# dojo-sim/ContactImplicitMPC.jl

Measured on AMD Instinct MI355X. Metric: MPC steps/s (quadruped, H=40, fp64), higher is better.
Workload: dtype f64

## Files before the change

### contactimplicitmpc/jl_amd/csrc/cimpc_host.cpp

```cpp
#include <hip/hip_runtime.h>

#include <algorithm>
#include <chrono>
#include <cmath>
#include <cstdio>
#include <cstdlib>
#include <cstring>
#include <string>
#include <vector>

#include "cimpc_internal.h"
#include "lin_table.h"
#include "lin_table_build.h"
#include "model_table.h"
#include "newton_state.h"
#include "gains.h"
#include "handle_state.h"
#include "plant_linearize.h"
#include "schedule_plan.h"

using namespace cimpc;

namespace {

thread_local std::string g_create_error;

enum ProfClass { PC_IP = 0, PC_KKT = 1, PC_RESID = 2, PC_OTHER = 3, PC_ASYNC = 4, PC_COUNT = 5 };

struct ProfRec {
    hipEvent_t a, b;
    int cls;
};

}

struct RoundStreams {
    hipStream_t st = nullptr;
    hipStream_t st_kkt = nullptr;
    hipEvent_t ev_join = nullptr;
    hipEvent_t ev_start = nullptr;
};

struct Knobs {
    SchedulePolicy sched{};
    bool async_debug = false;
    double watchdog_s = 30.0;
    bool debug_rounds = false;
    bool generic_static = false;
    KktPolicy kkt{};
    int kkt_tw_nb = 0;
    int kkt_tw_spins = 0;
    int banded_form = 0;

    static int env_int(const char* name, int dflt) { const char* v = getenv(name); return v ? atoi(v) : dflt; }
    void read_environment() {
        sched.async_mode = env_int("CIMPC_ASYNC", sched.async_mode);
        sched.async_tail = env_int("CIMPC_ASYNC_TAIL", sched.async_tail);
        sched.spec_first = env_int("CIMPC_SPEC_FIRST", sched.spec_first);
        sched.iter_cap = std::max(1, env_int("CIMPC_ITER_CAP", sched.iter_cap));
        async_debug = getenv("CIMPC_ASYNC_DEBUG") != nullptr;
        if (const char* v = getenv("CIMPC_ASYNC_WATCHDOG_S")) watchdog_s = atof(v);
        debug_rounds = getenv("CIMPC_DEBUG_ROUNDS") != nullptr;
        sched.tail_div = env_int("CIMPC_TAIL_DIV", sched.tail_div);
        sched.async_full_max = env_int("CIMPC_ASYNC_FULL_MAX", sched.async_full_max);
        sched.drain_pct = env_int("CIMPC_DRAIN_PCT", sched.drain_pct);
        sched.drain_min = std::max(1, env_int("CIMPC_DRAIN_MIN", sched.drain_min));
        kkt.kkt_pipe = env_int("CIMPC_KKT_PIPE", kkt.kkt_pipe);
        kkt.kkt_twisted = env_int("CIMPC_KKT_TWISTED", kkt.kkt_twisted);
        kkt_tw_nb = env_int("CIMPC_KKT_TW_NB", kkt_tw_nb);
        kkt.lazy_dz = env_int("CIMPC_LAZY_DZ", 1) != 0;
        kkt.kkt_duo = env_int("CIMPC_KKT_DUO", kkt.kkt_duo);
        kkt.kkt_duo_hint = env_int("CIMPC_KKT_DUO_HINT", kkt.kkt_duo_hint);
        kkt.async_kkt_tw = env_int("CIMPC_ASYNC_KKT_TW", kkt.async_kkt_tw);
        generic_static = env_int("CIMPC_GENERIC_STATIC", generic_static ? 1 : 0) != 0;
        sched.sweep_wgs = env_int("CIMPC_SWEEP_WGS", sched.sweep_wgs);
        sched.waves32 = env_int("CIMPC_WAVES32", sched.waves32);
        banded_form = env_int("CIMPC_BANDED_FORM", banded_form);
    }
};

struct cimpc_ctx {
    cimpc_dims dm{};
    Knobs kn{};
    cimpc_ip_opts ip{};
    cimpc_newton_opts nt{};
    int device = 0;
    hipStream_t stream = nullptr;
    bool own_stream = false;
    std::string err;
    KernelInfo ki{};
    int nz = 0, nth = 0, nths = 0, nd = 0, nr = 0, nx = 0, ny = 0, N = 0;
    std::vector<void*> allocs;
    double* d_tab = nullptr;
    IpQueues Q{};
    int* d_window = nullptr;
    double *g_q = nullptr, *g_u = nullptr, *g_w = nullptr, *g_g = nullptr, *g_b = nullptr, *g_th = nullptr, *g_stride = nullptr;
    int* g_phase = nullptr;
    int* d_good_src = nullptr;
    double* d_dz_knot = nullptr;
    double* d_alt = nullptr;
    double* d_zout = nullptr;
    double *d_Q = nullptr, *d_R = nullptr, *d_Qinv = nullptr, *d_Rinv = nullptr, *d_Cg = nullptr,
           *d_Cb = nullptr;
    double *d_q0 = nullptr, *d_q1 = nullptr;
    double* h_qin = nullptr;
    double* h_stage = nullptr;
    size_t h_stage_doubles = 0;
    double* d_result = nullptr;
    double* h_result = nullptr;
    double* d_rhs = nullptr;
    double* d_pstate = nullptr;
    long long ip_budget_ticks = 0;
    NewtonDev S{};
    int* h_counters = nullptr;
    std::vector<char> knot_set;
    int n_knots_set = 0;
    HandleState st;
    KktPolicy kp{};
    KktCaps kc{};
    KktBackend kb = KktBackend::Condensed;
    long long n_kkt_twisted = 0;
    int* h_twfail = nullptr;
    int twfail_seen = 0;
    long long n_kkt_tw_fallbacks = 0;
    bool band_reduce_ok = false;
    double* d_mix_ws = nullptr;
    int* d_mix_nfb = nullptr;
    size_t dense_ws_doubles = 0;
    bool cf_tiny = true;
    double* d_cf_ws = nullptr;
    double* d_dense_ws = nullptr;
    double *d_V = nullptr, *d_qt = nullptr, *d_vt = nullptr;
    int* d_ring = nullptr;
    size_t ctl_ints = 0;
    int* h_ring = nullptr;
    int* h_ring_dev = nullptr;
    SchedulePlan sched{};
    bool async_dirty = true;
    int* a_items = nullptr;
    int* a_jobs = nullptr;
    int* a_ctrl = nullptr;
    int* a_evals = nullptr;
    long long* a_dbg = nullptr;
    size_t a_cap = 0, a_rq_cap = 0, a_kq_cap = 0;
    RoundStreams rs;
    bool external_stream = false;
    std::vector<double> h_tab;
    std::vector<double> h_tab_work;
    double* d_tb = nullptr;
    size_t tb_cap = 0;
    double *d_gK = nullptr, *d_glatch = nullptr, *d_gio = nullptr;
    cimpc_stats last_stats{};
    int prof_on = 0;
    bool prof_open = false;
    std::vector<ProfRec> prof_recs;
    std::vector<hipEvent_t> ev_pool;
    double prof_ms[PC_COUNT] = {0, 0, 0, 0, 0};
    long long prof_n[PC_COUNT] = {0, 0, 0, 0, 0};
    long long prof_async_problems = 0;
    long long prof_ip_problems = 0, prof_kkt_systems = 0;
};

namespace {

int fail(cimpc_ctx* h, int code, const std::string& msg) {
    if (h) h->err = msg;
    else g_create_error = msg;
    return code;
}
int refuse(cimpc_ctx* h, const Refusal& r) { return r.code == CIMPC_OK ? CIMPC_OK : fail(h, r.code, r.msg); }

}

void cimpc::set_global_error(const std::string& msg) { g_create_error = msg; }

namespace {

#define HIP_TRY(h, call)                                                                     \
    do {                                                                                     \
        hipError_t e__ = (call);                                                             \
        if (e__ != hipSuccess)                                                               \
            return fail(h, CIMPC_ERR_HIP, std::string(#call) + ": " + hipGetErrorString(e__)); \
    } while (0)

template <class T>
int dev_alloc(cimpc_ctx* h, T** p, size_t count) {
    void* v = nullptr;
    if (count == 0) count = 1;
    hipError_t e = hipMalloc(&v, count * sizeof(T));
    if (e != hipSuccess) return fail(h, CIMPC_ERR_HIP, std::string("hipMalloc: ") + hipGetErrorString(e));
    e = hipMemset(v, 0, count * sizeof(T));
    if (e == hipSuccess) e = hipStreamSynchronize(nullptr);
    if (e != hipSuccess) return fail(h, CIMPC_ERR_HIP, std::string("hipMemset: ") + hipGetErrorString(e));
    h->allocs.push_back(v);
    *p = static_cast<T*>(v);
    return CIMPC_OK;
}

int table_layout(cimpc_ctx* h, LinLayout* L) {
    *L = LinLayout(h->nx, h->ny, h->nth, h->ki.G, h->ki.generic ? 0 : h->nths, h->ki.generic ? 0 : h->ki.adj);
    if (L->size != h->ki.tab_size) return fail(h, CIMPC_ERR_STATE, "table layout of the library and of the kernel differ");
    return CIMPC_OK;
}

void prof_begin(cimpc_ctx* h, int cls, hipStream_t st = nullptr) {
    h->prof_open = false;
    if (!h->prof_on || (h->prof_on == 2 && cls != PC_IP)) return;
    h->prof_open = true;
    if (!st) st = h->stream;
    ProfRec r;
    auto get = [&]() {
        if (!h->ev_pool.empty()) {
            hipEvent_t e = h->ev_pool.back();
            h->ev_pool.pop_back();
            return e;
        }
        hipEvent_t e;
        (void)hipEventCreate(&e);
        return e;
    };
    r.a = get();
    r.b = get();
    r.cls = cls;
    (void)hipEventRecord(r.a, st);
    h->prof_recs.push_back(r);
}
void prof_end(cimpc_ctx* h, hipStream_t st = nullptr) {
    if (!h->prof_on || !h->prof_open) return;
    h->prof_open = false;
    (void)hipEventRecord(h->prof_recs.back().b, st ? st : h->stream);
}
void prof_collect(cimpc_ctx* h) {
    if (h->prof_recs.empty()) return;
    (void)hipStreamSynchronize(h->stream);
    if (h->rs.st) (void)hipStreamSynchronize(h->rs.st);
    if (h->rs.st_kkt) (void)hipStreamSynchronize(h->rs.st_kkt);
    for (auto& r : h->prof_recs) {
        float ms = 0.f;
        if (hipEventElapsedTime(&ms, r.a, r.b) == hipSuccess) {
            h->prof_ms[r.cls] += ms;
            h->prof_n[r.cls] += 1;
        }
        h->ev_pool.push_back(r.a);
        h->ev_pool.push_back(r.b);
    }
    h->prof_recs.clear();
}

IpParams make_ip_params(cimpc_ctx* h, const TrajDev& T, int par, int* pending_counter, double* zout) {
    IpParams p{};
    p.tab = h->d_tab;
    p.Q = h->Q;
    p.Q.par = par;
    p.wpk = h->sched.wpk;
    p.q = T.q;
    p.theta = T.th;
    p.gam = T.g;
    p.bfr = T.b;
    p.alt = h->st.has_altitude() ? h->d_alt : nullptr;
    p.d = h->S.d;
    p.dz = h->S.dz;
    p.nu = nullptr; p.dtn = nullptr; p.dtn_ld = h->S.dtn_ld;
    p.status = h->S.ip_status;
    p.iters = h->S.ip_iters;
    p.zout = zout;
    p.pflag = h->S.pflag;
    p.pstate = h->d_pstate;
    p.pending_count = pending_counter;
    p.iter_cap = h->kn.sched.iter_cap;
    p.slots = CS;
    p.H = h->dm.H;
    p.o = h->ip;
    p.kc_floor = h->ip.kappa_tol / h->ip.undercut;
    p.tau_floor = 1.0 - h->ip.eps_min;
    p.reg_floor = h->ip.kappa_tol * h->ip.gamma_reg;
    p.budget_ticks = h->ip_budget_ticks;
    p.generic_static = h->kn.generic_static ? 1 : 0;
    return p;
}

int run_sweep(cimpc_ctx* h, int par, int* pending_counter, double* zout, hipStream_t st, int iter_cap = 0, int* drain_counter = nullptr,
              bool with_products = false, long long hint = -1) {
    IpParams p = make_ip_params(h, h->S.cand, par, pending_counter, zout);
    if (with_products && h->S.dtn != nullptr) { p.nu = h->S.nu_cand; p.dtn = h->S.dtn; }
    if (iter_cap > 0) p.iter_cap = iter_cap;
    const SweepLaunch l = plan_sweep(h->kn.sched, h->sched, hint, p.iter_cap, h->ip.max_iter, drain_counter != nullptr);
    p.wpk = l.wpk; p.direct = l.direct;
    if (l.drain_thresh > 0) { p.drain_count = drain_counter; p.drain_thresh = l.drain_thresh; p.drain_min = h->kn.sched.drain_min; }
    prof_begin(h, PC_IP, st);
    int rc = launch_ip_sweep(&h->dm, p, l.waves, st);
    prof_end(h, st);
    if (rc != CIMPC_OK) return fail(h, rc, "ip sweep launch failed");
    return CIMPC_OK;
}

static void set_kkt_backend(cimpc_ctx* h) {
    NewtonDev& S = h->S;
    KktCaps& c = h->kc;
    c.cfg = h->dm.mode == CIMPC_MODE_CONFIGURATION;
    c.velocity = S.V != nullptr;
    c.cf_tiny = h->cf_tiny;
    c.wide_tiles = (h->dm.nq > 16 || h->dm.nu > 16) && h->dm.nq <= 24 && h->dm.nu <= 24;
    c.condensed = kkt_condensed_available(S);
    c.mfma = kkt_mfma_available(S);
    c.packed = kkt_packed_available(S);
    c.twisted = kkt_twisted_available(S);
    c.duo = kkt_duo_available(S);
    c.mixed = kkt_mixed_available(S);
    auto pick_band_form = [&](auto avail) {
        for (int r = h->band_reduce_ok ? 1 : 0; r >= 0; --r) { S.band_reduce = r; if (avail()) return true; }
        S.band_reduce = h->band_reduce_ok ? 1 : 0;
        return false;
    };
    S.band_reduce = h->band_reduce_ok ? 1 : 0;
    c.banded = c.cfg && pick_band_form([&] { return kkt_banded_available(S); });
    c.cf_reduce = !c.cfg && (c.velocity ? pick_band_form([&] { return kkt_cf_reduce_available(S); }) : kkt_cf_reduce_available(S));
    c.banded_twisted = kkt_banded_twisted_available(c.cfg ? S : cf_shadow(S));
    h->kb = select_kkt_backend(c, h->nt.kkt_backend);
    S.good_src = kkt_lazy_commit(h->kp, c, h->kb) ? h->d_good_src : nullptr;
}

int ensure_kkt_ws(cimpc_ctx* h) {
    if (h->kb == KktBackend::Condensed) return CIMPC_OK;
    if (h->kb == KktBackend::CondensedMixed) {
        if (h->d_mix_ws) return CIMPC_OK;
        if (dev_alloc(h, &h->d_mix_ws, kkt_mixed_workspace_doubles(h->S)) != CIMPC_OK) return CIMPC_ERR_HIP;
        return dev_alloc(h, &h->d_mix_nfb, 1);
    }
    const bool cf = h->kb == KktBackend::CfCondensed || h->kb == KktBackend::CfBanded;
    if (cf && !h->d_cf_ws && dev_alloc(h, &h->d_cf_ws, cf_reduce_doubles(h->S)) != CIMPC_OK) return CIMPC_ERR_HIP;
    if (h->kb == KktBackend::CfCondensed) return CIMPC_OK;
    const size_t need = cf ? kkt_dense_workspace_doubles(cf_shadow(h->S), true) : kkt_dense_workspace_doubles(h->S, h->kb == KktBackend::Banded);
    if (h->d_dense_ws && h->dense_ws_doubles >= need) return CIMPC_OK;
    h->d_dense_ws = nullptr;
    h->dense_ws_doubles = need;
    return dev_alloc(h, &h->d_dense_ws, need);
}

static KktForm plan_kkt_stage(cimpc_ctx* h, const KktSite& site) {
    const KktForm f = choose_kkt_form(h->kp, h->kc, h->kb, site);
    if (two_ended(f)) h->n_kkt_twisted++;
    return f;
}
static int run_kkt_stage(cimpc_ctx* h, const NewtonDev& Sk, const KktArgs& K, const KktSite& site, const int* list, int n, const int* n_dev, hipStream_t st) {
    return launch_kkt_stage(Sk, K, h->kb, plan_kkt_stage(h, site), list, n, n_dev, KktWorkspace{h->d_dense_ws, h->d_cf_ws, h->d_mix_ws, h->d_mix_nfb}, st);
}

int read_stats(cimpc_ctx* h, long long out[4]) {
    std::vector<long long> v((size_t)h->dm.B * 4);
    HIP_TRY(h, hipMemcpy(v.data(), h->S.stats, v.size() * sizeof(long long), hipMemcpyDeviceToHost));
    out[0] = out[1] = out[2] = out[3] = 0;
    for (size_t b = 0; b < (size_t)h->dm.B; ++b)
        for (int k = 0; k < 4; ++k) out[k] += v[b * 4 + k];
    return CIMPC_OK;
}

int drain_pending(cimpc_ctx* h) {
    if (!h->st.drain_needed()) return CIMPC_OK;
    HIP_TRY(h, hipStreamSynchronize(h->stream));
    h->st.advance_drained();
    return CIMPC_OK;
}

int check_ready(cimpc_ctx* h, bool need_newton) {
    if (!h) return CIMPC_ERR_INVALID;
    return refuse(h, h->st.solve_refusal(h->n_knots_set == h->dm.H_ref, need_newton));
}

}

extern "C" {

int cimpc_version(void) { return 108; }

void cimpc_default_ip_opts(cimpc_ip_opts* o) {
    if (!o) return;
    o->r_tol = 1.0e-8;
    o->kappa_tol = 2.0e-4;
    o->undercut = 5.0;
    o->gamma_reg = 0.1;
    o->kappa_reg = 1.0e-3;
    o->eps_min = 0.05;
    o->ls_scale = 0.5;
    o->max_iter = 100;
    o->max_ls = 3;
    o->stall_alpha = 1.0e-13;
    o->max_time = 0.0;
}

void cimpc_default_newton_opts(cimpc_newton_opts* o) {
    if (!o) return;
    o->r_tol = 3.0e-4;
    o->beta_init = 1.0e-5;
    o->max_time = 0.0;
    o->kappa = 2.0e-4;
    o->max_iter = 5;
    o->kkt_backend = CIMPC_KKT_CONDENSED;
}

const char* cimpc_last_error(cimpc_handle h) { return h ? h->err.c_str() : g_create_error.c_str(); }

int cimpc_create(const cimpc_dims* dims, const cimpc_ip_opts* ip, const cimpc_newton_opts* nt,
                 int device, cimpc_handle* out) {
    if (!dims || !out) return fail(nullptr, CIMPC_ERR_INVALID, "null argument");
    *out = nullptr;
    const cimpc_dims& d = *dims;
    if (d.nq <= 0 || d.nu < 0 || d.nw < 0 || d.nc <= 0 || d.nb < 0 || d.H <= 0 || d.H_ref <= 0 ||
        d.B <= 0 || (d.mode != 0 && d.mode != 1))
        return fail(nullptr, CIMPC_ERR_INVALID, "invalid dimensions");
    int ndev = 0;
    if (hipGetDeviceCount(&ndev) != hipSuccess || ndev <= 0)
        return fail(nullptr, CIMPC_ERR_NO_DEVICE,
                    "no HIP device visible: this library has no CPU fallback");
    if (device < 0 || device >= ndev) return fail(nullptr, CIMPC_ERR_NO_DEVICE, "device index out of range");
    hipDeviceProp_t prop;
    if (hipGetDeviceProperties(&prop, device) != hipSuccess)
        return fail(nullptr, CIMPC_ERR_NO_DEVICE, "hipGetDeviceProperties failed");
    if (std::strncmp(prop.gcnArchName, "gfx950", 6) != 0)
        return fail(nullptr, CIMPC_ERR_NO_DEVICE,
                    std::string("device is ") + prop.gcnArchName + ", kernels are built for gfx950 only");
    if (hipSetDevice(device) != hipSuccess) return fail(nullptr, CIMPC_ERR_NO_DEVICE, "hipSetDevice failed");

    cimpc_ctx* h = new cimpc_ctx();
    h->dm = d;
    if (ip) h->ip = *ip; else cimpc_default_ip_opts(&h->ip);
    if (nt) h->nt = *nt; else cimpc_default_newton_opts(&h->nt);
    h->device = device;
    if (h->ip.max_time > 0.0 && h->ip.max_time < 1000.0) {
        if (h->ip.max_iter >= 128) { delete h; return fail(nullptr, CIMPC_ERR_INVALID, "ip max_time needs max_iter < 128 (the parked state packs both into one word)"); }
        int khz = 0;
        if (hipDeviceGetAttribute(&khz, hipDeviceAttributeWallClockRate, device) != hipSuccess || khz <= 0) {
            delete h;
            return fail(nullptr, CIMPC_ERR_HIP, "ip max_time: the device does not report hipDeviceAttributeWallClockRate");
        }
        h->ip_budget_ticks = std::max<long long>(1, (long long)std::llround(h->ip.max_time * 1.0e3 * (double)khz));
    }
    h->kn.read_environment();
    if (ip_kernel_info(&h->dm, &h->ki) != CIMPC_OK) {
        delete h;
        std::string built;
        for (const ModelRow& r : MODEL_TABLE) (built += built.empty() ? "" : ", ") += r.name;
        return fail(nullptr, CIMPC_ERR_INVALID, "model dimensions outside the runtime-dimension kernel (nx, ny <= 64) and without a compiled set (built: " + built + ")");
    }
    h->nx = d.nq;
    h->ny = 2 * d.nc + d.nb;
    h->nz = d.nq + 4 * d.nc + 2 * d.nb;
    h->nth = 2 * d.nq + d.nu + d.nw + 2;
    h->nths = 2 * d.nq + d.nu;
    h->nd = d.mode ? d.nq + d.nc + d.nb : d.nq;
    h->nr = d.mode ? d.nq + d.nu + d.nc + d.nb : d.nq + d.nu;
    h->N = d.H * (h->nr + h->nd);
    if (hipStreamCreateWithFlags(&h->stream, hipStreamNonBlocking) != hipSuccess) {
        delete h;
        return fail(nullptr, CIMPC_ERR_HIP, "hipStreamCreate failed");
    }
    h->own_stream = true;
    h->knot_set.assign(d.H_ref, 0);
    h->h_tab.assign(h->ki.tab_size, 0.0);
    h->h_tab_work.assign(lin_table_work_doubles(h->nx, h->ny), 0.0);

    const size_t B = d.B, H = d.H;
    int rc = CIMPC_OK;
    {
        const size_t K = d.H_ref;
        const size_t evals = 1 + 7 * (size_t)std::max(1, h->nt.max_iter);
        h->a_cap = B * evals * ((H + K - 1) / K + 1);
        h->a_rq_cap = B * (2 + 3 * (size_t)std::max(1, h->nt.max_iter));
        h->a_kq_cap = B * (2 + 3 * (size_t)std::max(1, h->nt.max_iter));
        const size_t bytes = (K * h->a_cap + h->a_rq_cap + h->a_kq_cap) * sizeof(int);
        h->sched = plan_schedule(h->kn.sched, ScheduleFacts{d.B, d.H, d.H_ref, h->ki.G, newton_async_available(&d) && K <= 256 && bytes <= ((size_t)1 << 30)});
    }
    auto A = [&](auto** p, size_t n) { if (rc == CIMPC_OK) rc = dev_alloc(h, p, n); };
    A(&h->d_tab, (size_t)d.H_ref * h->ki.tab_size);
    {
        const size_t K = d.H_ref;
        const size_t cap = B * CS * ((H + K - 1) / K + 1);
        h->Q.K = (int)K; h->Q.cap = (int)cap; h->Q.par = 0;
        A(&h->Q.items, 2 * K * cap);
        const QueueCtl L = queue_ctl(K);
        h->ctl_ints = L.ints;
        A(&h->Q.count, h->ctl_ints);
        if (rc == CIMPC_OK) { h->Q.head = h->Q.count + L.head; h->d_ring = h->Q.count + L.counters; }
        A(&h->Q.done_count, B * CS);
        A(&h->d_window, B * (H + 2));
        h->Q.window = h->d_window;
    }
    A(&h->d_alt, B * d.nc);
    A(&h->d_zout, B * CS * H * h->nz);
    A(&h->d_Q, H * d.nq * d.nq);
    A(&h->d_R, H * d.nu * d.nu);
    A(&h->d_Qinv, H * d.nq * d.nq);
    A(&h->d_Rinv, H * d.nu * d.nu);
    A(&h->d_Cg, H * d.nc * d.nc);
    A(&h->d_Cb, H * d.nb * d.nb);
    A(&h->d_V, H * d.nq * d.nq);
    A(&h->d_qt, H * d.nq);
    A(&h->d_vt, H * d.nq);
    A(&h->d_q0, 2 * B * d.nq);
    if (rc == CIMPC_OK) h->d_q1 = h->d_q0 + B * d.nq;
    A(&h->d_result, result_doubles(B, d.nu));
    if (rc == CIMPC_OK && (hipHostMalloc((void**)&h->h_qin, (2 * B + 1) * d.nq * sizeof(double), hipHostMallocDefault) != hipSuccess ||
                           hipHostMalloc((void**)&h->h_result, result_doubles(B, d.nu) * sizeof(double), hipHostMallocDefault) != hipSuccess))
        rc = CIMPC_ERR_HIP;
    A(&h->d_rhs, B * h->N);
    NewtonDev& S = h->S;
    S.dm = d;
    S.b0 = 0;
    S.nb_launch = d.B;
    S.nd = h->nd; S.nr = h->nr; S.nth = h->nth; S.nths = h->nths; S.N = h->N;
    const size_t BS = B * CS;
    for (TrajDev* T : {&S.traj, &S.cand, &S.ref}) {
        const size_t n = (T == &S.cand) ? BS : B;
        A(&T->q, n * (H + 2) * d.nq); A(&T->u, n * H * d.nu); A(&T->w, n * H * d.nw);
        A(&T->g, n * H * d.nc); A(&T->b, n * H * d.nb); A(&T->th, n * H * h->nth);
    }
    A(&S.nu, B * H * h->nd); A(&S.nu_cand, BS * H * h->nd); A(&S.d, BS * H * h->nd);
    A(&S.dz, BS * H * h->nths * h->nd); A(&S.dz_good, B * H * h->nths * h->nd); A(&h->d_good_src, B * H);
    S.dtn_ld = h->ki.generic ? 0 : h->ki.dtn_ld;
    if (S.dtn_ld > 0) A(&S.dtn, BS * H * (size_t)S.dtn_ld);
    A(&S.ip_status, BS * H); A(&S.ip_iters, BS * H); A(&S.pflag, BS * H); A(&S.cur_slot, B);
    A(&h->d_pstate, BS * H * (2 * (size_t)h->nx + 4 * (size_t)h->ny + 4));
    A(&S.res, B * h->N); A(&S.res_cand, BS * h->N); A(&S.delta, B * h->N);
    A(&S.r_norm, B); A(&S.r_cand, BS); A(&S.alpha, B); A(&S.beta, B);
    A(&S.ls_iter, B); A(&S.newton_l, B); A(&S.stage, B); A(&S.need_sweep, BS);
    A(&S.kkt_list, 2 * B);
    A(&S.slot_list, 2 * BS);
    A(&S.counters, ROUND_COUNTER_INTS);
    A(&S.stats, std::max<size_t>(B * 4, 64));
    A(&S.ro_sweeps, B); A(&S.ro_ip_iters, B); A(&S.ro_ip_fail, B); A(&S.nlog, B * NLOG * 4);
    A(&S.kkt_ws, B * H * (3 * (size_t)h->nd * h->nd + h->nd));
    A(&S.kkt_tw_xch, B * kkt_tw_xch_doubles(h->nd));
    A(&S.kkt_tw_flags, B * KKT_TW_FLAGS);
    if (rc == CIMPC_OK && hipHostMalloc((void**)&h->h_counters, ROUND_COUNTER_INTS * sizeof(int)) != hipSuccess)
        rc = fail(h, CIMPC_ERR_HIP, "hipHostMalloc failed");
    if (rc != CIMPC_OK) {
        g_create_error = h->err;
        cimpc_destroy(h);
        return rc;
    }
    S.Q = h->d_Q; S.R = h->d_R; S.Qinv = h->d_Qinv; S.Rinv = h->d_Rinv; S.Cg = h->d_Cg; S.Cb = h->d_Cb;
    if (hipMemset(h->d_good_src, 0xFF, B * H * sizeof(int)) != hipSuccess || hipStreamSynchronize(nullptr) != hipSuccess) {
        g_create_error = "hipMemset failed"; cimpc_destroy(h); return CIMPC_ERR_HIP;
    }
    S.band_form = h->kn.banded_form;
    S.r_tol = h->nt.r_tol; S.beta_init = h->nt.beta_init; S.kappa = h->nt.kappa; S.max_iter = h->nt.max_iter;
    h->kp = h->kn.kkt;
    h->kp.kkt_overlap = h->sched.kkt_overlap;
    set_kkt_backend(h);
    S.spec_all = h->sched.spec_all; S.spec_first = h->sched.spec_first; S.spec_mid = h->sched.spec_mid;
    S.kkt_tw_nb = h->kn.kkt_tw_nb;
    S.kkt_tw_epoch = 0;
    S.kkt_tw_spins = h->kn.kkt_tw_spins > 0 ? h->kn.kkt_tw_spins : KKT_TW_SPINS;
    {
        int* dv = nullptr;
        if (hipHostMalloc((void**)&h->h_twfail, 4 * sizeof(int), hipHostMallocMapped) != hipSuccess ||
            hipHostGetDevicePointer((void**)&dv, h->h_twfail, 0) != hipSuccess) {
            g_create_error = "mapped counter allocation failed"; cimpc_destroy(h); return CIMPC_ERR_HIP;
        }
        h->h_twfail[0] = 0;
        S.kkt_tw_fail = dv;
    }
    if (hipHostMalloc((void**)&h->h_ring, RING_ALLOC_INTS * sizeof(int), hipHostMallocMapped) != hipSuccess ||
        hipHostGetDevicePointer((void**)&h->h_ring_dev, h->h_ring, 0) != hipSuccess) {
        g_create_error = "ring allocation failed"; cimpc_destroy(h); return CIMPC_ERR_HIP;
    }
    if (h->sched.async_on) {
        const size_t K = d.H_ref;
        if (dev_alloc(h, &h->a_items, K * h->a_cap) != CIMPC_OK || dev_alloc(h, &h->a_jobs, h->a_rq_cap + h->a_kq_cap) != CIMPC_OK ||
            dev_alloc(h, &h->a_ctrl, async_ctl(K).ints) != CIMPC_OK || dev_alloc(h, &h->a_evals, B) != CIMPC_OK) {
            g_create_error = h->err; cimpc_destroy(h); return CIMPC_ERR_HIP;
        }
        if (h->kn.async_debug && dev_alloc(h, &h->a_dbg, 16) != CIMPC_OK) { g_create_error = h->err; cimpc_destroy(h); return CIMPC_ERR_HIP; }
        h->async_dirty = true;
    }
    {
        RoundStreams& r = h->rs;
        if (hipStreamCreateWithFlags(&r.st, hipStreamNonBlocking) != hipSuccess ||
            hipStreamCreateWithFlags(&r.st_kkt, hipStreamNonBlocking) != hipSuccess ||
            hipEventCreateWithFlags(&r.ev_join, hipEventDisableTiming) != hipSuccess ||
            hipEventCreateWithFlags(&r.ev_start, hipEventDisableTiming) != hipSuccess) {
            g_create_error = "stream creation failed"; cimpc_destroy(h); return CIMPC_ERR_HIP;
        }
    }
    *out = h;
    return CIMPC_OK;
}

int cimpc_destroy(cimpc_handle h) {
    if (!h) return CIMPC_ERR_INVALID;
    (void)hipSetDevice(h->device);
    if (h->stream) (void)hipStreamSynchronize(h->stream);
    for (auto& r : h->prof_recs) { (void)hipEventDestroy(r.a); (void)hipEventDestroy(r.b); }
    for (auto e : h->ev_pool) (void)hipEventDestroy(e);
    for (void* p : h->allocs) (void)hipFree(p);
    if (h->d_tb) (void)hipFree(h->d_tb);
    if (h->h_counters) (void)hipHostFree(h->h_counters);
    if (h->h_ring) (void)hipHostFree(h->h_ring);
    if (h->h_qin) (void)hipHostFree(h->h_qin);
    if (h->h_result) (void)hipHostFree(h->h_result);
    if (h->h_stage) (void)hipHostFree(h->h_stage);
    if (h->h_twfail) (void)hipHostFree(h->h_twfail);
    {
        RoundStreams& r = h->rs;
        if (r.st) { (void)hipStreamSynchronize(r.st); (void)hipStreamDestroy(r.st); }
        if (r.st_kkt) { (void)hipStreamSynchronize(r.st_kkt); (void)hipStreamDestroy(r.st_kkt); }
        if (r.ev_join) (void)hipEventDestroy(r.ev_join);
        if (r.ev_start) (void)hipEventDestroy(r.ev_start);
    }
    if (h->own_stream && h->stream) (void)hipStreamDestroy(h->stream);
    delete h;
    return CIMPC_OK;
}

int cimpc_set_stream(cimpc_handle h, void* hip_stream) {
    if (!h) return CIMPC_ERR_INVALID;
    (void)hipStreamSynchronize(h->stream);
    h->st.advance_drained();
    if (h->own_stream && h->stream) (void)hipStreamDestroy(h->stream);
    h->stream = static_cast<hipStream_t>(hip_stream);
    h->own_stream = false;
    h->external_stream = true;
    return CIMPC_OK;
}

int cimpc_synchronize(cimpc_handle h) {
    if (!h) return CIMPC_ERR_INVALID;
    HIP_TRY(h, hipStreamSynchronize(h->stream));
    return CIMPC_OK;
}

int cimpc_set_linearization(cimpc_handle h, int t, const double* z0, const double* th0,
                            const double* r0, const double* rz0, const double* rth0) {
    if (!h || !z0 || !th0 || !r0 || !rz0 || !rth0) return fail(h, CIMPC_ERR_INVALID, "null argument");
    if (t < 1 || t > h->dm.H_ref) return fail(h, CIMPC_ERR_INVALID, "knot index out of range (1-based)");
    if (int dp = drain_pending(h); dp != CIMPC_OK) return dp;
    LinLayout L(0, 0, 0, 0);
    if (int rc = table_layout(h, &L); rc != CIMPC_OK) return rc;
    if (!lin_table_build_knot(L, z0, th0, r0, rz0, rth0, h->h_tab_work.data(), h->h_tab.data(), SoloTeam{}))
        return fail(h, CIMPC_ERR_INVALID, "Dx = rz0[idyn, ix] is singular");
    HIP_TRY(h, hipSetDevice(h->device));
    HIP_TRY(h, hipMemcpy(h->d_tab + (size_t)(t - 1) * L.size, h->h_tab.data(), (size_t)L.size * sizeof(double),
                         hipMemcpyHostToDevice));
    if (!h->knot_set[t - 1]) { h->knot_set[t - 1] = 1; h->n_knots_set++; }
    return CIMPC_OK;
}

namespace {

int build_tables_on_device(cimpc_ctx* h, int t0, int N, const double* z0, const double* th0, const double* r0, const double* rz0,
                           const double* rth0, int model, int n_ter_up, int n_terrain, const cimpc_terrain* terrain, double kappa) {
    if (int dp = drain_pending(h); dp != CIMPC_OK) return dp;
    const size_t nz = h->nz, nth = h->nth;
    LinLayout L(0, 0, 0, 0);
    if (int rc = table_layout(h, &L); rc != CIMPC_OK) return rc;
    constexpr size_t TW = sizeof(cimpc_terrain) / sizeof(double);
    const size_t n_z = (size_t)N * nz, n_th = (size_t)N * nth, n_ter = (size_t)n_ter_up * TW;
    const size_t o_th = n_z, o_ter = o_th + n_th, o_r = o_ter + n_ter, o_rz = o_r + n_z, o_rth = o_rz + n_z * nz;
    const size_t o_tab = o_rth + n_z * nth, o_st = o_tab + (size_t)N * L.size, total = o_st + ((size_t)N + 1) / 2;
    const size_t n_up = model >= 0 ? o_r : o_tab;
    std::vector<double> up(n_up);
    std::memcpy(up.data(), z0, n_z * sizeof(double));
    std::memcpy(up.data() + o_th, th0, n_th * sizeof(double));
    if (n_ter) std::memcpy(up.data() + o_ter, terrain, n_ter * sizeof(double));
    if (model < 0) {
        std::memcpy(up.data() + o_r, r0, n_z * sizeof(double));
        std::memcpy(up.data() + o_rz, rz0, n_z * nz * sizeof(double));
        std::memcpy(up.data() + o_rth, rth0, n_z * nth * sizeof(double));
    }
    HIP_TRY(h, hipSetDevice(h->device));
    if (h->tb_cap < total) {
        if (h->d_tb) (void)hipFree(h->d_tb);
        h->d_tb = nullptr; h->tb_cap = 0;
        HIP_TRY(h, hipMalloc((void**)&h->d_tb, total * sizeof(double)));
        h->tb_cap = total;
    }
    double* D = h->d_tb;
    int* d_status = reinterpret_cast<int*>(D + o_st);
    hipStream_t st = h->stream;
    HIP_TRY(h, hipMemcpyAsync(D, up.data(), n_up * sizeof(double), hipMemcpyHostToDevice, st));
    bool launched = true;
    if (model >= 0)
        launched = plant_linearize_launch(model, N, D, D + o_th, n_ter ? reinterpret_cast<const cimpc_terrain*>(D + o_ter) : nullptr, n_terrain,
                                          kappa, D + o_r, D + o_rz, D + o_rth, st);
    launched = launched && lin_table_build_launch(L, N, D, D + o_th, D + o_r, D + o_rz, D + o_rth, D + o_tab, d_status, st);
    if (!launched) {
        (void)hipStreamSynchronize(st);
        return fail(h, CIMPC_ERR_HIP, "the table build could not be launched");
    }
    std::vector<int> status(N);
    HIP_TRY(h, hipMemcpyAsync(status.data(), d_status, (size_t)N * sizeof(int), hipMemcpyDeviceToHost, st));
    HIP_TRY(h, hipStreamSynchronize(st));
    for (int k = 0; k < N; ++k)
        if (status[k] != 0) return fail(h, CIMPC_ERR_INVALID, "Dx = rz0[idyn, ix] is singular at knot " + std::to_string(t0 + k) + "; no knot was changed");
    HIP_TRY(h, hipMemcpyAsync(h->d_tab + (size_t)(t0 - 1) * L.size, D + o_tab, (size_t)N * L.size * sizeof(double), hipMemcpyDeviceToDevice, st));
    HIP_TRY(h, hipStreamSynchronize(st));
    for (int t = t0; t < t0 + N; ++t)
        if (!h->knot_set[t - 1]) { h->knot_set[t - 1] = 1; h->n_knots_set++; }
    return CIMPC_OK;
}

}

int cimpc_set_linearization_batch(cimpc_handle h, int t0, int N, const double* z0, const double* th0,
                                  const double* r0, const double* rz0, const double* rth0) {
    if (!h || !z0 || !th0 || !r0 || !rz0 || !rth0) return fail(h, CIMPC_ERR_INVALID, "null argument");
    if (t0 < 1 || N < 1 || N > h->dm.H_ref || t0 - 1 > h->dm.H_ref - N) return fail(h, CIMPC_ERR_INVALID, "knot range out of the table (1-based)");
    return build_tables_on_device(h, t0, N, z0, th0, r0, rz0, rth0, -1, 0, 0, nullptr, 0.0);
}

int cimpc_linearize_knots(cimpc_handle h, int model, int t0, int N, int n_terrain, const cimpc_terrain* terrain,
                          const double* z, const double* theta, double kappa) {
    if (!h || !z || !theta) return fail(h, CIMPC_ERR_INVALID, "null argument");
    if (t0 < 1 || N < 1 || N > h->dm.H_ref || t0 - 1 > h->dm.H_ref - N) return fail(h, CIMPC_ERR_INVALID, "knot range out of the table (1-based)");
    PlantLinearizeDims pd{};
    if (plant_linearize_check(model, N, n_terrain, terrain, z, theta, kappa, &pd) != CIMPC_OK)
        return fail(h, CIMPC_ERR_INVALID, "cimpc_plant_linearize would refuse these arguments");
    const cimpc_dims& d = h->dm;
    if (pd.nq != d.nq || pd.nu != d.nu || pd.nw != d.nw || pd.nc != d.nc || pd.nb != d.nb)
        return fail(h, CIMPC_ERR_INVALID, "the plant model's (nq, nu, nw, nc, nb) are not the handle's");
    return build_tables_on_device(h, t0, N, z, theta, nullptr, nullptr, nullptr, model, pd.n_terrain_up, n_terrain, terrain, kappa);
}

int cimpc_get_table(cimpc_handle h, int t, double* table) {
    if (!h || !table) return fail(h, CIMPC_ERR_INVALID, "null argument");
    if (t < 1 || t > h->dm.H_ref) return fail(h, CIMPC_ERR_INVALID, "knot index out of range (1-based)");
    if (int dp = drain_pending(h); dp != CIMPC_OK) return dp;
    LinLayout L(0, 0, 0, 0);
    if (int rc = table_layout(h, &L); rc != CIMPC_OK) return rc;
    HIP_TRY(h, hipSetDevice(h->device));
    HIP_TRY(h, hipMemcpy(table, h->d_tab + (size_t)(t - 1) * L.size, (size_t)L.size * sizeof(double), hipMemcpyDeviceToHost));
    return CIMPC_OK;
}

int cimpc_set_objective(cimpc_handle h, const double* Q, const double* R, const double* Cg,
                        const double* Cb, const double* V, const double* q_target,
                        const double* v_target) {
    if (!h || !Q || !R) return fail(h, CIMPC_ERR_INVALID, "Q and R are required");
    const cimpc_dims& d = h->dm;
    const size_t H = d.H;
    {
        auto symmetric = [&](const double* A, int n) {
            for (size_t t = 0; t < H; ++t) {
                const double* M = A + t * n * n;
                double amax = 0.0, asym = 0.0;
                for (int i = 0; i < n; ++i)
                    for (int j = 0; j < n; ++j) { amax = std::max(amax, std::fabs(M[i + j * n])); asym = std::max(asym, std::fabs(M[i + j * n] - M[j + i * n])); }
                if (asym > 1e-9 * amax) return false;
            }
            return true;
        };
        const bool lu = h->nt.kkt_backend == CIMPC_KKT_DENSE_LU;
        if (!lu && !symmetric(Q, d.nq)) return fail(h, CIMPC_ERR_INVALID, "objective block Q[i] is not symmetric");
        if (!lu && d.nu > 0 && !symmetric(R, d.nu)) return fail(h, CIMPC_ERR_INVALID, "objective block R[i] is not symmetric");
        if (!lu && V && !symmetric(V, d.nq)) return fail(h, CIMPC_ERR_INVALID, "objective block V[i] is not symmetric");
    }
    HIP_TRY(h, hipSetDevice(h->device));
    if (int dp = drain_pending(h); dp != CIMPC_OK) return dp;
    {
        double gmax = 0.0;
        if (Cg) for (size_t k = 0; k < H * d.nc * d.nc; ++k) gmax = std::max(gmax, std::fabs(Cg[k]));
        if (Cb) for (size_t k = 0; k < H * d.nb * d.nb; ++k) gmax = std::max(gmax, std::fabs(Cb[k]));
        h->cf_tiny = gmax <= 1e-30;
    }
    if (V != nullptr) {
        std::vector<double> vt(H * d.nq, 0.0), qt(H * d.nq, 0.0);
        if (v_target) std::copy(v_target, v_target + H * d.nq, vt.begin());
        if (q_target) std::copy(q_target, q_target + H * d.nq, qt.begin());
        else {
            bool any = false;
            for (double x : vt) any = any || x != 0.0;
            if (any) for (size_t t = 1; t < H; ++t) for (int k = 0; k < d.nq; ++k) qt[t * d.nq + k] = qt[(t - 1) * d.nq + k] + vt[(t - 1) * d.nq + k];
        }
        HIP_TRY(h, hipMemcpy(h->d_V, V, H * d.nq * d.nq * sizeof(double), hipMemcpyHostToDevice));
        HIP_TRY(h, hipMemcpy(h->d_qt, qt.data(), qt.size() * sizeof(double), hipMemcpyHostToDevice));
        HIP_TRY(h, hipMemcpy(h->d_vt, vt.data(), vt.size() * sizeof(double), hipMemcpyHostToDevice));
        h->S.V = h->d_V; h->S.q_target = h->d_qt; h->S.v_target = h->d_vt;
    } else {
        h->S.V = nullptr; h->S.q_target = nullptr; h->S.v_target = nullptr;
    }
    std::vector<double> Qi(H * d.nq * d.nq), Ri(H * d.nu * d.nu), work(lin_invert_work_doubles(std::max(d.nq, d.nu)));
    auto inverse = [&](const double* A, double* Ai, int n) {
        if (!lin_invert(A, n, n, work.data(), SoloTeam{})) return false;
        for (int c = 0; c < n; ++c)
            for (int r = 0; r < n; ++r) Ai[r + (size_t)c * n] = work[(size_t)r * 2 * n + n + c];
        return true;
    };
    bool q_inverted = true, r_inverted = true;
    for (size_t i = 0; i < H; ++i) {
        if (!inverse(Q + i * d.nq * d.nq, Qi.data() + i * d.nq * d.nq, d.nq)) q_inverted = false;
        if (d.nu > 0 && !inverse(R + i * d.nu * d.nu, Ri.data() + i * d.nu * d.nu, d.nu)) r_inverted = false;
    }
    h->band_reduce_ok = r_inverted && d.nu > 0 && (h->kn.banded_form & 4) == 0;
    set_kkt_backend(h);
    const bool need_inv = h->kb == KktBackend::Condensed || h->kb == KktBackend::CondensedMixed || h->kb == KktBackend::CfCondensed;
    if (need_inv && !q_inverted) { h->st.objective_refused(); return fail(h, CIMPC_ERR_INVALID, "objective block Q[i] is singular"); }
    if (need_inv && !r_inverted) { h->st.objective_refused(); return fail(h, CIMPC_ERR_INVALID, "objective block R[i] is singular"); }
    HIP_TRY(h, hipMemcpy(h->d_Q, Q, H * d.nq * d.nq * sizeof(double), hipMemcpyHostToDevice));
    HIP_TRY(h, hipMemcpy(h->d_R, R, H * d.nu * d.nu * sizeof(double), hipMemcpyHostToDevice));
    HIP_TRY(h, hipMemcpy(h->d_Qinv, Qi.data(), Qi.size() * sizeof(double), hipMemcpyHostToDevice));
    HIP_TRY(h, hipMemcpy(h->d_Rinv, Ri.data(), Ri.size() * sizeof(double), hipMemcpyHostToDevice));
    if (Cg) HIP_TRY(h, hipMemcpy(h->d_Cg, Cg, H * d.nc * d.nc * sizeof(double), hipMemcpyHostToDevice));
    if (Cb) HIP_TRY(h, hipMemcpy(h->d_Cb, Cb, H * d.nb * d.nb * sizeof(double), hipMemcpyHostToDevice));
    h->st.objective_replaced();
    return CIMPC_OK;
}

int cimpc_set_altitude(cimpc_handle h, const double* alt) {
    if (!h) return CIMPC_ERR_INVALID;
    if (!alt) { h->st.altitude_cleared(); return CIMPC_OK; }
    HIP_TRY(h, hipSetDevice(h->device));
    if (int dp = drain_pending(h); dp != CIMPC_OK) return dp;
    HIP_TRY(h, hipMemcpy(h->d_alt, alt, (size_t)h->dm.B * h->dm.nc * sizeof(double), hipMemcpyHostToDevice));
    h->st.altitude_set();
    return CIMPC_OK;
}

static int sync_dz_stores(cimpc_ctx* h, int next_producer) {
    if (!h->st.dz_sync_needed(next_producer)) return CIMPC_OK;
    const size_t row = (size_t)h->dm.H * h->nths * h->nd * sizeof(double), B = h->dm.B;
    if (next_producer == DZ_IMPLICIT)
        HIP_TRY(h, hipMemcpy2DAsync(h->S.dz, CS * row, h->S.dz_good, row, row, B, hipMemcpyDeviceToDevice, h->stream));
    else
        HIP_TRY(h, hipMemcpy2DAsync(h->S.dz_good, row, h->S.dz, CS * row, row, B, hipMemcpyDeviceToDevice, h->stream));
    HIP_TRY(h, hipStreamSynchronize(h->stream));
    return CIMPC_OK;
}

static int rekey_out(cimpc_ctx* h) {
    if (!h->st.rekey_out_needed()) return CIMPC_OK;
    if (!h->d_dz_knot && dev_alloc(h, &h->d_dz_knot, (size_t)h->dm.B * h->dm.H_ref * h->nths * h->nd) != CIMPC_OK) return CIMPC_ERR_HIP;
    int rc = launch_dz_rekey(h->S, h->d_dz_knot, h->d_window, h->st.rekey_out_store(), 0, h->stream);
    return rc == CIMPC_OK ? CIMPC_OK : fail(h, rc, "sensitivity archive launch failed");
}
static int rekey_in(cimpc_ctx* h) {
    if (!h->st.rekey_in_needed(h->d_dz_knot != nullptr)) return CIMPC_OK;
    for (int which = 0; which < 2; ++which) {
        int rc = launch_dz_rekey(h->S, h->d_dz_knot, h->d_window, which, 1, h->stream);
        if (rc != CIMPC_OK) return fail(h, rc, "sensitivity restore launch failed");
    }
    return CIMPC_OK;
}

static int then_sync(cimpc_ctx* h, int rc) {
    if (rc != CIMPC_OK) return rc;
    HIP_TRY(h, hipStreamSynchronize(h->stream));
    return CIMPC_OK;
}

int cimpc_set_window(cimpc_handle h, const int* window) {
    if (!h || !window) return fail(h, CIMPC_ERR_INVALID, "null argument");
    h->st.unlatch();
    std::vector<int> w0(horizon_sizes(h->dm, h->nth, h->nd).win);
    if (int rc = refuse(h, window_to_knots(window, w0.size(), h->dm.H_ref, w0.data())); rc != CIMPC_OK) return rc;
    HIP_TRY(h, hipSetDevice(h->device));
    if (int dp = drain_pending(h); dp != CIMPC_OK) return dp;
    return window_move(h->st, WindowHome::Host, w0.data(), w0.size(),
        [&] { return then_sync(h, rekey_out(h)); },
        [&]() -> int { HIP_TRY(h, hipMemcpy(h->d_window, w0.data(), w0.size() * sizeof(int), hipMemcpyHostToDevice)); return CIMPC_OK; },
        [&] { return then_sync(h, rekey_in(h)); });
}

int cimpc_set_reference(cimpc_handle h, const double* q_ref, const double* u_ref,
                        const double* w_ref, const double* gamma_ref, const double* b_ref,
                        const double* theta_ref) {
    if (!h || !q_ref || !u_ref || !theta_ref) return fail(h, CIMPC_ERR_INVALID, "q_ref, u_ref, theta_ref are required");
    h->st.unlatch();
    const HorizonSizes n = horizon_sizes(h->dm, h->nth, h->nd);
    HIP_TRY(h, hipSetDevice(h->device));
    if (int dp = drain_pending(h); dp != CIMPC_OK) return dp;
    HIP_TRY(h, hipMemcpy(h->S.ref.q, q_ref, n.q * sizeof(double), hipMemcpyHostToDevice));
    HIP_TRY(h, hipMemcpy(h->S.ref.u, u_ref, n.u * sizeof(double), hipMemcpyHostToDevice));
    if (w_ref) HIP_TRY(h, hipMemcpy(h->S.ref.w, w_ref, n.w * sizeof(double), hipMemcpyHostToDevice));
    else {
        HIP_TRY(h, hipMemset(h->S.ref.w, 0, n.w * sizeof(double)));
        HIP_TRY(h, hipStreamSynchronize(nullptr));
    }
    if (gamma_ref) HIP_TRY(h, hipMemcpy(h->S.ref.g, gamma_ref, n.g * sizeof(double), hipMemcpyHostToDevice));
    if (b_ref) HIP_TRY(h, hipMemcpy(h->S.ref.b, b_ref, n.b * sizeof(double), hipMemcpyHostToDevice));
    HIP_TRY(h, hipMemcpy(h->S.ref.th, theta_ref, n.th * sizeof(double), hipMemcpyHostToDevice));
    h->st.reference_replaced();
    return CIMPC_OK;
}

int cimpc_implicit_dynamics(cimpc_handle h, const double* q, const double* theta,
                            const double* gamma, const double* b, double* d_out, double* dz,
                            int* status, int* iters, double* z) {
    int rc = check_ready(h, false);
    if (rc != CIMPC_OK) return rc;
    if (!q || !theta) return fail(h, CIMPC_ERR_INVALID, "q and theta are required");
    const cimpc_dims& d = h->dm;
    const size_t B = d.B, H = d.H;
    const HorizonSizes row = horizon_rows(d, h->nth, h->nd);
    if (d.mode == CIMPC_MODE_CONFIGURATIONFORCE && (!gamma || !b))
        return fail(h, CIMPC_ERR_INVALID, "gamma and b are required in configurationforce mode");
    HIP_TRY(h, hipSetDevice(h->device));
    if (int sy = sync_dz_stores(h, DZ_IMPLICIT); sy != CIMPC_OK) return sy;
    h->st.implicit_dynamics_started();
    TrajDev& T = h->S.cand;
    auto up = [&](double* dst, const double* src, size_t row_doubles) {
        return hipMemcpy2DAsync(dst, CS * row_doubles * sizeof(double), src, row_doubles * sizeof(double),
                                row_doubles * sizeof(double), B, hipMemcpyHostToDevice, h->stream);
    };
    HIP_TRY(h, up(T.q, q, row.q));
    HIP_TRY(h, up(T.th, theta, row.th));
    if (gamma) HIP_TRY(h, up(T.g, gamma, row.g));
    if (b) HIP_TRY(h, up(T.b, b, row.b));
    HIP_TRY(h, hipMemsetAsync(h->Q.count, 0, 2 * h->Q.K * QPAD * sizeof(int), h->stream));
    HIP_TRY(h, hipMemsetAsync(h->Q.head, 0, h->Q.K * QPAD * sizeof(int), h->stream));
    {
        NewtonDev Sk = h->S;
        Sk.WQ = h->Q; Sk.WQ.par = 0;
        rc = launch_enqueue_all(Sk, h->stream);
        if (rc != CIMPC_OK) return fail(h, rc, "enqueue launch failed");
    }
    for (int pass = 0; pass < 64; ++pass) {
        const int par = pass & 1;
        HIP_TRY(h, hipMemsetAsync(h->S.counters, 0, ROUND_COUNTER_INTS * sizeof(int), h->stream));
        rc = run_sweep(h, par, round_counter(h->S.counters, RC_PARKED), z ? h->d_zout : nullptr, h->stream);
        if (rc != CIMPC_OK) return rc;
        HIP_TRY(h, hipMemsetAsync(h->Q.count + (size_t)par * h->Q.K * QPAD, 0, h->Q.K * QPAD * sizeof(int), h->stream));
        HIP_TRY(h, hipMemsetAsync(h->Q.head, 0, h->Q.K * QPAD * sizeof(int), h->stream));
        HIP_TRY(h, hipMemcpyAsync(h->h_counters, round_counter(h->S.counters, RC_PARKED), sizeof(int), hipMemcpyDeviceToHost, h->stream));
        HIP_TRY(h, hipStreamSynchronize(h->stream));
        if (*h->h_counters == 0) break;
    }
    auto down = [&](void* dst, const void* src, size_t row_bytes) {
        return hipMemcpy2DAsync(dst, row_bytes, src, CS * row_bytes, row_bytes, B, hipMemcpyDeviceToHost, h->stream);
    };
    if (d_out) HIP_TRY(h, down(d_out, h->S.d, row.nu * sizeof(double)));
    if (dz) HIP_TRY(h, down(dz, h->S.dz, H * h->nths * h->nd * sizeof(double)));
    if (status) HIP_TRY(h, down(status, h->S.ip_status, H * sizeof(int)));
    if (iters) HIP_TRY(h, down(iters, h->S.ip_iters, H * sizeof(int)));
    if (z) HIP_TRY(h, down(z, h->d_zout, H * h->nz * sizeof(double)));
    HIP_TRY(h, hipStreamSynchronize(h->stream));
    return CIMPC_OK;
}

static int run_ip_callback(cimpc_handle h, int t, int n, int op, const double* z, const double* theta, const double* alt,
                           const double* r, double kappa, double reg, double* out) {
    if (!h || !z || !out || n <= 0) return fail(h, CIMPC_ERR_INVALID, "null argument");
    if (t < 1 || t > h->dm.H_ref) return fail(h, CIMPC_ERR_INVALID, "knot index out of range (1-based)");
    if (!h->knot_set[t - 1]) return fail(h, CIMPC_ERR_STATE, "set_linearization has not been called for this knot");
    if (h->ki.generic) return fail(h, CIMPC_ERR_INVALID, "B2 callbacks exist for the compiled lane-group models only");
    HIP_TRY(h, hipSetDevice(h->device));
    const size_t nz = h->nz, nth = h->nth, nc = h->dm.nc;
    const size_t naux = std::max(nz, nth);
    const size_t tot = (size_t)n * (2 * nz + naux + nc);
    double* buf = nullptr;
    HIP_TRY(h, hipMalloc((void**)&buf, tot * sizeof(double)));
    double* d_z = buf; double* d_out = buf + (size_t)n * nz; double* d_aux = d_out + (size_t)n * nz; double* d_alt = d_aux + (size_t)n * naux;
    auto done = [&](int rc) { (void)hipFree(buf); return rc; };
    if (hipMemcpy(d_z, z, (size_t)n * nz * sizeof(double), hipMemcpyHostToDevice) != hipSuccess) return done(fail(h, CIMPC_ERR_HIP, "upload failed"));
    const double* aux = op == 0 ? theta : r;
    if (!aux) return done(fail(h, CIMPC_ERR_INVALID, "null argument"));
    if (hipMemcpy(d_aux, aux, (size_t)n * (op == 0 ? nth : nz) * sizeof(double), hipMemcpyHostToDevice) != hipSuccess) return done(fail(h, CIMPC_ERR_HIP, "upload failed"));
    if (alt && hipMemcpy(d_alt, alt, (size_t)n * nc * sizeof(double), hipMemcpyHostToDevice) != hipSuccess) return done(fail(h, CIMPC_ERR_HIP, "upload failed"));
    IpCallbackArgs a{};
    a.tab = h->d_tab; a.knot = t - 1; a.n = n; a.op = op; a.z = d_z;
    a.theta = op == 0 ? d_aux : nullptr; a.alt = (op == 0 && alt) ? d_alt : nullptr; a.r = op == 1 ? d_aux : nullptr;
    a.kappa = kappa; a.reg = reg; a.out = d_out;
    (void)hipGetLastError();
    const int rc = launch_ip_callback(&h->dm, a, h->stream);
    if (rc != CIMPC_OK) return done(fail(h, rc, "callback launch failed"));
    if (hipStreamSynchronize(h->stream) != hipSuccess ||
        hipMemcpy(out, d_out, (size_t)n * nz * sizeof(double), hipMemcpyDeviceToHost) != hipSuccess) return done(fail(h, CIMPC_ERR_HIP, "callback kernel failed"));
    return done(CIMPC_OK);
}

int cimpc_ip_residual(cimpc_handle h, int t, int n, const double* z, const double* theta, const double* alt, double kappa, double* r) {
    return run_ip_callback(h, t, n, 0, z, theta, alt, nullptr, kappa, 0.0, r);
}

int cimpc_ip_linear_solve(cimpc_handle h, int t, int n, const double* z, const double* r, double reg, double* delta) {
    return run_ip_callback(h, t, n, 1, z, nullptr, nullptr, r, 0.0, reg, delta);
}

int cimpc_kkt_solve(cimpc_handle h, const double* r, double beta, double* delta) {
    int rc = check_ready(h, true);
    if (rc != CIMPC_OK) return rc;
    if (!r || !delta) return fail(h, CIMPC_ERR_INVALID, "null argument");
    const size_t n = (size_t)h->dm.B * h->N;
    HIP_TRY(h, hipSetDevice(h->device));
    HIP_TRY(h, hipMemcpyAsync(h->d_rhs, r, n * sizeof(double), hipMemcpyHostToDevice, h->stream));
    if ((rc = ensure_kkt_ws(h)) != CIMPC_OK) return rc;
    for (int attempt = 0; attempt < 2; ++attempt) {
        h->S.kkt_tw_epoch += 1;
        const int fails0 = *(volatile int*)h->h_twfail;
        prof_begin(h, PC_KKT);
        rc = run_kkt_stage(h, h->S, kkt_raw_args(h->d_rhs, beta, h->S.delta), KktSite{.kind = KktSite::Seam, .attempt = attempt, .B = h->dm.B},
                           nullptr, h->S.nb_launch, nullptr, h->stream);
        prof_end(h);
        if (rc != CIMPC_OK) return fail(h, rc, "kkt launch failed");
        HIP_TRY(h, hipMemcpyAsync(delta, h->S.delta, n * sizeof(double), hipMemcpyDeviceToHost, h->stream));
        HIP_TRY(h, hipStreamSynchronize(h->stream));
        const int fails1 = *(volatile int*)h->h_twfail;
        if (fails1 == fails0) break;
        h->n_kkt_tw_fallbacks += fails1 - fails0;
        h->twfail_seen = fails1;
    }
    return CIMPC_OK;
}

int cimpc_kkt_solve_rho(cimpc_handle h, const double* r, double rho, double* delta) {
    if (!h) return CIMPC_ERR_INVALID;
    if (!(rho >= 0.0) || !(h->nt.kappa > 0.0)) return fail(h, CIMPC_ERR_INVALID, "rho must be >= 0 (and kappa > 0)");
    const double Hk = (double)h->dm.H, kap = h->nt.kappa;
    auto f = [&](double b) { return Hk * b * kap; };
    double beta = rho / (Hk * kap), err = std::fabs(f(beta) - rho), lo = beta, hi = beta;
    for (int k = 0; k < 4 && err != 0.0; ++k) {
        lo = std::nextafter(lo, -HUGE_VAL); hi = std::nextafter(hi, HUGE_VAL);
        for (double c : {lo, hi}) { const double e = std::fabs(f(c) - rho); if (e < err) { err = e; beta = c; } }
    }
    return cimpc_kkt_solve(h, r, beta, delta);
}

namespace {

struct RoundCounts { int sweep, kkt, slots, new_slots, parked, finished; };
RoundCounts read_round_counts(const int* ring, long long round) {
    const volatile int* hr = ring_slot((const volatile int*)ring, round);
    return {hr[RING_N_SWEEP], hr[RING_N_KKT], hr[RING_SLOTS], hr[RING_NEW_SLOTS], hr[RING_PARKED], hr[RING_FINISHED]};
}

struct SolveRun {
    const double *q0_dev, *q1_dev; int warm_start;
    std::chrono::steady_clock::time_point t0;
    int tw_fail0;
    bool hybrid;
    RoundStreams sb;
    RoundCounts last;
};

bool has_time_budget(const cimpc_ctx* h) { return h->nt.max_time > 0.0 && h->nt.max_time < 1.0e6; }
double elapsed_s(const SolveRun& run) { return std::chrono::duration<double>(std::chrono::steady_clock::now() - run.t0).count(); }
bool over_budget(const cimpc_ctx* h, const SolveRun& run) { return h->nt.max_time > 0.0 && elapsed_s(run) >= h->nt.max_time; }
int note_tw_fallbacks(cimpc_ctx* h) {
    const int cur = *(volatile int*)h->h_twfail;
    if (cur != h->twfail_seen) { h->n_kkt_tw_fallbacks += cur - h->twfail_seen; h->twfail_seen = cur; }
    return cur;
}

NewtonDev launch_view(const cimpc_ctx* h, int parity) {
    NewtonDev Sk = h->S;
    Sk.b0 = 0; Sk.nb_launch = h->dm.B;
    Sk.counters = round_counter_block(h->d_ring, parity);
    Sk.counters_next = round_counter_block(h->d_ring, parity ^ 1);
    Sk.host_flag = ring_slot(h->h_ring_dev, parity);
    Sk.WQ = h->Q; Sk.WQ.par = parity;
    return Sk;
}
void wire_async_queues(const cimpc_ctx* h, NewtonDev& Sk) {
    const AsyncCtl L = async_ctl(h->Q.K);
    int* const c = h->a_ctrl;
    Sk.WQ.items = h->a_items; Sk.WQ.cap = (int)h->a_cap; Sk.WQ.count = c + L.count; Sk.WQ.head = c + L.head;
    AsyncQ& A = Sk.A;
    A.on = 1;
    A.rq_items = h->a_jobs; A.rq_head = c + L.rq_head; A.rq_tail = c + L.rq_tail;
    A.kq_items = h->a_jobs + h->a_rq_cap; A.kq_head = c + L.kq_head; A.kq_tail = c + L.kq_tail;
    A.n_done = c + L.n_done; A.epoch = c + L.epoch; A.evals_left = h->a_evals;
    A.abort_flag = ring_abort_word((volatile int*)h->h_ring_dev);
}

int finish_results(cimpc_ctx* h, hipStream_t st) {
    if (launch_dz_commit(h->S, st) != CIMPC_OK) return fail(h, CIMPC_ERR_HIP, "sensitivity flush launch failed");
    if (int rf = launch_solve_finish(h->S, h->d_result, st); rf != CIMPC_OK) return fail(h, rf, "result kernel launch failed");
    HIP_TRY(h, hipMemcpyAsync(h->h_result, h->d_result, result_doubles(h->dm.B, h->dm.nu) * sizeof(double), hipMemcpyDeviceToHost, st));
    return CIMPC_OK;
}
void publish_stats(cimpc_ctx* h, long long rounds) {
    const double* r = h->h_result;
    cimpc_stats& s = h->last_stats;
    s.sweeps = (long long)r[RESULT_SWEEPS]; s.ip_solves = (long long)r[RESULT_IP_SOLVES];
    s.ip_iters = (long long)r[RESULT_IP_ITERS]; s.ip_failures = (long long)r[RESULT_IP_FAILURES];
    s.rounds = rounds; s.newton_iters = (long long)r[RESULT_NEWTON_SUM];
}

int print_async_debug(cimpc_ctx* h) {
    long long dv[16];
    HIP_TRY(h, hipMemcpy(dv, h->a_dbg, sizeof(dv), hipMemcpyDeviceToHost));
    fprintf(stderr, "[cimpc async] WG-ms: other %.2f kkt %.2f resid %.2f ip %.2f | jobs: kkt %lld resid %lld serve %lld | grid %d service %d | group-trips %.2fM active %.1f%% | group-ms pop %.1f fence %.1f | pop: cas %lld spins %lld claim-ms %.1f wait-ms %.1f\n",
            dv[0] * 1e-5, dv[1] * 1e-5, dv[2] * 1e-5, dv[3] * 1e-5, dv[9], dv[10], dv[11], h->sched.async_grid, h->sched.async_service, dv[5] * 1e-6, dv[5] ? 100.0 * dv[4] / dv[5] : 0.0, dv[6] * 1e-5, dv[7] * 1e-5, dv[12], dv[13], dv[14] * 1e-5, dv[15] * 1e-5);
    return CIMPC_OK;
}
void print_queued_problems(cimpc_ctx* h, const SolveRun& run, long long r, int par, long long hint) {
    std::vector<int> qc((size_t)h->Q.K * QPAD);
    (void)hipStreamSynchronize(run.sb.st); (void)hipStreamSynchronize(run.sb.st_kkt);
    if (hipMemcpy(qc.data(), h->Q.count + (size_t)par * h->Q.K * QPAD, qc.size() * sizeof(int), hipMemcpyDeviceToHost) != hipSuccess) return;
    long long tot = 0;
    for (int k = 0; k < h->Q.K; ++k) tot += qc[(size_t)k * QPAD];
    fprintf(stderr, "[cimpc round %lld] sweep launch: %lld problems queued (host hint %lld)\n", r, tot, hint);
}

int run_async(cimpc_ctx* h, SolveRun& run, bool from_reset, long long rounds_before) {
    NewtonDev& S = h->S;
    IpQueues LQ = h->Q; LQ.par = (int)(rounds_before & 1);
    hipStream_t st = run.sb.st;
    if (h->async_dirty) {
        HIP_TRY(h, hipMemsetAsync(h->a_items, 0xFF, (size_t)h->Q.K * h->a_cap * sizeof(int), st));
        HIP_TRY(h, hipMemsetAsync(h->a_jobs, 0xFF, (h->a_rq_cap + h->a_kq_cap) * sizeof(int), st));
        h->async_dirty = false;
    }
    HIP_TRY(h, hipMemsetAsync(h->a_ctrl, 0, async_ctl(h->Q.K).ints * sizeof(int), st));
    volatile int* abort_word = ring_abort_word((volatile int*)h->h_ring);
    *abort_word = 0;
    NewtonDev Sk = launch_view(h, 0);
    if (!from_reset) Sk.spec_all = h->sched.spec_tail;
    wire_async_queues(h, Sk);
    AsyncQ& A = Sk.A;
    A.n_service = from_reset ? h->sched.async_service : h->sched.tail_service;
    A.idle_sleep = async_idle_sleep; A.idle_spins = async_idle_spins; A.wake_fan = async_wake_fan;
    A.dbg = h->a_dbg; A.B = h->dm.B;
    if (h->a_dbg) HIP_TRY(h, hipMemsetAsync(h->a_dbg, 0, 16 * sizeof(long long), st));
    const KktSite site{.kind = from_reset ? KktSite::Persistent : KktSite::HybridTail, .tw_off = *(volatile int*)h->h_twfail != run.tw_fail0,
                       .B = h->dm.B, .async_tail = h->sched.async_tail, .waves = std::min(h->sched.waves, 4)};
    A.kkt_tw = plan_kkt_stage(h, site) == KktForm::AsyncTwoJob ? 1 : 0;
    S.kkt_tw_epoch += h->nt.max_iter + 2;
    prof_begin(h, PC_OTHER, st);
    int rc2 = from_reset ? launch_reset(Sk, run.q0_dev, run.q1_dev, run.warm_start, st) : launch_async_handoff(Sk, LQ, st);
    prof_end(h, st);
    if (rc2 != CIMPC_OK) return fail(h, rc2, "reset / hand-off launch failed");
    IpParams p = make_ip_params(h, S.cand, 0, round_counter(h->d_ring, RC_PARKED), nullptr);
    if (S.dtn != nullptr) { p.nu = S.nu_cand; p.dtn = S.dtn; }
    p.Q = Sk.WQ;
    p.iter_cap = h->ip.max_iter + 1;
    p.A = A;
    long long solved_before = 0;
    if (h->prof_on && !from_reset) { long long sv[4]; if (int rs = read_stats(h, sv); rs != CIMPC_OK) return rs; solved_before = sv[1]; }
    prof_begin(h, PC_ASYNC, st);
    rc2 = launch_newton_async(&h->dm, p, Sk, std::min(h->sched.waves, 4), from_reset ? h->sched.async_grid : h->sched.tail_grid, st);
    prof_end(h, st);
    if (rc2 != CIMPC_OK) return fail(h, rc2, "asynchronous newton launch failed");
    if (int rf = finish_results(h, st); rf != CIMPC_OK) return rf;
    const bool budget = has_time_budget(h);
    bool timed_out = false; long long polls = 0;
    const auto tw = std::chrono::steady_clock::now();
    while (hipStreamQuery(st) == hipErrorNotReady) {
        const bool over = budget && over_budget(h, run);
        timed_out = !over && (++polls & 0x3FF) == 0 && std::chrono::duration<double>(std::chrono::steady_clock::now() - tw).count() > h->kn.watchdog_s;
        if (over || timed_out) { *abort_word = 1; h->async_dirty = true; break; }
    }
    HIP_TRY(h, hipStreamSynchronize(st));
    note_tw_fallbacks(h);
    if (timed_out) return fail(h, CIMPC_ERR_HIP, "asynchronous solve: watchdog expired (no completion within CIMPC_ASYNC_WATCHDOG_S)");
    if (h->a_dbg) { if (int rd = print_async_debug(h); rd != CIMPC_OK) return rd; }
    publish_stats(h, rounds_before + 1);
    h->prof_ip_problems += solved_before;
    h->prof_async_problems += h->last_stats.ip_solves - solved_before;
    if (from_reset) h->prof_kkt_systems += h->last_stats.newton_iters;
    return CIMPC_OK;
}

int launch_round(cimpc_ctx* h, SolveRun& run, long long r, bool blind) {
    const RoundStreams& sb = run.sb; const RoundCounts& last = run.last;
    const int par = (int)(r & 1);
    h->S.kkt_tw_epoch += 1;
    const bool tw_off = note_tw_fallbacks(h) != run.tw_fail0;
    NewtonDev Sk = launch_view(h, par);
    Sk.A.n_done = run.hybrid ? h->a_ctrl + async_ctl(h->Q.K).n_done : nullptr;
    Sk.round_stamp = (int)(r + 1);
    const bool kkt = (r > 0) && (blind || last.kkt > 0);
    const int n_kkt = blind ? h->dm.B : last.kkt;
    const int* n_kkt_dev = blind ? round_counter(Sk.counters_next, RC_KKT) : nullptr;
    if (kkt) {
        const bool ov = h->kp.kkt_overlap;
        const KktSite site{.kind = ov ? KktSite::Overlapped : KktSite::Round, .n_kkt = n_kkt, .blind = blind,
                           .sweep_problems = (long long)last.new_slots * h->dm.H, .tw_off = tw_off, .B = h->dm.B};
        hipStream_t kst = ov ? sb.st_kkt : sb.st;
        if (!ov) Sk.kkt_same_round = 1;
        prof_begin(h, PC_KKT, kst);
        int rk = run_kkt_stage(h, Sk, kkt_newton_args(Sk), site, Sk.kkt_list + (size_t)(par ^ 1) * h->dm.B,
                               ov ? last.kkt : n_kkt, ov ? nullptr : n_kkt_dev, kst);
        prof_end(h, kst);
        if (rk != CIMPC_OK) return fail(h, rk, "kkt launch failed");
        if (ov && hipEventRecord(sb.ev_join, sb.st_kkt) != hipSuccess) return fail(h, CIMPC_ERR_HIP, "join record failed");
    }
    const RoundPlan rp = plan_round(h->kn.sched, h->sched, h->ip.max_iter, kkt, blind, last.sweep, last.slots);
    const long long hint = blind ? -1 : (long long)last.slots * h->dm.H + last.parked;
    if (h->kn.debug_rounds && !blind) print_queued_problems(h, run, r, par, hint);
    int rr = run_sweep(h, par, round_counter(Sk.counters, RC_PARKED), nullptr, sb.st, rp.cap, round_counter(Sk.counters, RC_DRAINED), true, hint);
    if (rr != CIMPC_OK) return rr;
    prof_begin(h, PC_RESID, sb.st);
    if (rp.split_join) {
        rr = launch_resid_decide(Sk, sb.st, rp.n_slots, 1);
        if (rr != CIMPC_OK) return fail(h, rr, "residual launch failed");
    }
    if (kkt && h->kp.kkt_overlap && hipStreamWaitEvent(sb.st, sb.ev_join, 0) != hipSuccess) return fail(h, CIMPC_ERR_HIP, "join failed");
    rr = launch_resid_decide(Sk, sb.st, rp.n_slots, rp.split_join ? 2 : 0);
    prof_end(h, sb.st);
    if (rr != CIMPC_OK) return fail(h, rr, "residual launch failed");
    return CIMPC_OK;
}

}

int cimpc_newton_solve_dev(cimpc_handle h, const double* q0_dev, const double* q1_dev, int warm_start) {
    int rc = check_ready(h, true);
    if (rc != CIMPC_OK) return rc;
    if (!q0_dev || !q1_dev) return fail(h, CIMPC_ERR_INVALID, "null argument");
    HIP_TRY(h, hipSetDevice(h->device));
    if (int sy = sync_dz_stores(h, DZ_NEWTON); sy != CIMPC_OK) return sy;
    h->st.solve_started();
    const int B = h->dm.B;
    SolveRun run{q0_dev, q1_dev, warm_start, {}, *(volatile int*)h->h_twfail, false, h->rs, RoundCounts{B, 0, B, B, 0, 0}};
    h->twfail_seen = run.tw_fail0;
    run.t0 = std::chrono::steady_clock::now();
    RoundStreams& sb = run.sb;
    if (h->external_stream) sb.st = h->stream;
    else {
        HIP_TRY(h, hipEventRecord(sb.ev_start, h->stream));
        HIP_TRY(h, hipStreamWaitEvent(sb.st, sb.ev_start, 0));
    }
    HIP_TRY(h, hipMemsetAsync(h->S.stats, 0, (size_t)B * 4 * sizeof(long long), sb.st));
    if ((rc = ensure_kkt_ws(h)) != CIMPC_OK) return rc;
    const SolvePath path = choose_solve_path(h->sched, h->kb);
    if (path == SolvePath::Persistent) return run_async(h, run, true, 0);
    run.hybrid = path == SolvePath::Hybrid;
    const int round_limit = max_rounds(h->kn.sched, h->nt.max_iter, h->ip.max_iter);
    long long launched = 0, completed = 0;
    const bool ahead = round_ahead(h->sched, h->kb, warm_start != 0, has_time_budget(h));
    HIP_TRY(h, hipMemsetAsync(h->Q.count, 0, h->ctl_ints * sizeof(int), sb.st));
    if (run.hybrid) HIP_TRY(h, hipMemsetAsync(h->a_ctrl + async_ctl(h->Q.K).jobs, 0, ASYNC_JOB_INTS * sizeof(int), sb.st));
    for (int slot = 0; slot < RING_SLOTS_COUNT; ++slot) ring_slot((volatile int*)h->h_ring, slot)[RING_STAMP] = 0;
    prof_begin(h, PC_OTHER, sb.st);
    rc = launch_reset(launch_view(h, 0), q0_dev, q1_dev, warm_start, sb.st);
    prof_end(h, sb.st);
    if (rc != CIMPC_OK) return fail(h, rc, "reset launch failed");
    while (true) {
        if (completed >= round_limit) {
            (void)hipStreamSynchronize(sb.st); (void)hipStreamSynchronize(sb.st_kkt);
            return fail(h, CIMPC_ERR_STATE, "newton_solve: round limit reached with unfinished rollouts");
        }
        while (launched <= completed + (ahead ? 1 : 0)) {
            rc = launch_round(h, run, launched, launched > completed);
            if (rc != CIMPC_OK) return rc;
            ++launched;
        }
        {
            volatile int* hm = ring_slot((volatile int*)h->h_ring, completed);
            const int want = (int)(completed + 1);
            long long spins = 0;
            while (hm[RING_STAMP] != want) {
                if ((++spins & 0xFFFFF) == 0 && hipStreamQuery(sb.st) != hipErrorNotReady && hm[RING_STAMP] != want)
                    return fail(h, CIMPC_ERR_HIP, "round finished without publishing its counters");
            }
        }
        const RoundCounts& last = run.last = read_round_counts(h->h_ring, completed);
        if (h->kn.debug_rounds) fprintf(stderr, "[cimpc round %lld] t %.3f ms: next sweep %d rollouts (%d evaluation slots), next kkt %d, parked %d, finished %d\n", completed,
                                        1e3 * elapsed_s(run), last.sweep, last.slots, last.kkt, last.parked, last.finished);
        h->prof_kkt_systems += last.kkt;
        ++completed;
        if ((last.sweep == 0 && last.kkt == 0) || over_budget(h, run)) break;
        if (run.hybrid && hand_over(h->sched, B - last.finished)) {
            HIP_TRY(h, hipStreamSynchronize(sb.st));
            HIP_TRY(h, hipStreamSynchronize(sb.st_kkt));
            return run_async(h, run, false, completed);
        }
    }
    HIP_TRY(h, hipStreamSynchronize(sb.st_kkt));
    if (int rf = finish_results(h, sb.st); rf != CIMPC_OK) return rf;
    HIP_TRY(h, hipStreamSynchronize(sb.st));
    publish_stats(h, completed);
    h->prof_ip_problems += h->last_stats.ip_solves;
    return CIMPC_OK;
}

int cimpc_newton_solve(cimpc_handle h, const double* q0, const double* q1, int warm_start,
                       double* u1, int* newton_iters, double* r_norm) {
    if (!h || !q0 || !q1) return fail(h, CIMPC_ERR_INVALID, "null argument");
    const size_t ne = (size_t)h->dm.B * h->dm.nq;
    HIP_TRY(h, hipSetDevice(h->device));
    std::memcpy(h->h_qin, q0, ne * sizeof(double));
    std::memcpy(h->h_qin + ne, q1, ne * sizeof(double));
    HIP_TRY(h, hipMemcpyAsync(h->d_q0, h->h_qin, 2 * ne * sizeof(double), hipMemcpyHostToDevice, h->stream));
    int rc = cimpc_newton_solve_dev(h, h->d_q0, h->d_q1, warm_start);
    if (rc != CIMPC_OK) return rc;
    const int nu = h->dm.nu;
    for (int b = 0; b < h->dm.B; ++b) {
        const double* o = h->h_result + result_u1(b, nu);
        if (u1) std::memcpy(u1 + (size_t)b * nu, o, nu * sizeof(double));
        if (newton_iters) newton_iters[b] = (int)o[record_iters(nu)];
        if (r_norm) r_norm[b] = o[record_r_norm(nu)] / (double)h->N;
    }
    return CIMPC_OK;
}

int cimpc_mpc_solve(cimpc_handle h, const int* window, const double* q_ref, const double* u_ref, const double* w_ref,
                    const double* gamma_ref, const double* b_ref, const double* theta_ref, const double* alt,
                    const double* q0, const double* q1, int warm_start, double* u1, int* newton_iters, double* r_norm,
                    double* q, double* u, double* gamma, double* b, double* nu_dual) {
    if (!h || !q0 || !q1) return fail(h, CIMPC_ERR_INVALID, "null argument");
    if (q_ref && (!u_ref || !theta_ref)) return fail(h, CIMPC_ERR_INVALID, "q_ref, u_ref, theta_ref go together");
    const HorizonSizes sz = horizon_sizes(h->dm, h->nth, h->nd);
    HIP_TRY(h, hipSetDevice(h->device));
    if (!h->h_stage) {
        h->h_stage_doubles = (sz.win + 1) / 2 + sz.q + sz.u + sz.w + sz.g + sz.b + std::max(sz.th, sz.nu) + sz.alt + 8;
        if (hipHostMalloc((void**)&h->h_stage, h->h_stage_doubles * sizeof(double), hipHostMallocDefault) != hipSuccess)
            return fail(h, CIMPC_ERR_HIP, "hipHostMalloc failed");
    }
    if (int dp = drain_pending(h); dp != CIMPC_OK) return dp;
    double* stage = h->h_stage;
    int* s_win = reinterpret_cast<int*>(stage);
    double* s_q = stage + (sz.win + 1) / 2; double* s_u = s_q + sz.q; double* s_w = s_u + sz.u; double* s_g = s_w + sz.w;
    double* s_b = s_g + sz.g; double* s_th = s_b + sz.b; double* s_alt = s_th + std::max(sz.th, sz.nu);
    hipStream_t st = h->stream;
    if (window) {
        if (int rc = refuse(h, window_to_knots(window, sz.win, h->dm.H_ref, s_win)); rc != CIMPC_OK) return rc;
        if (!h->st.mirror_equals(s_win, sz.win)) {
            int rc = window_move(h->st, WindowHome::Host, s_win, sz.win, [&] { return rekey_out(h); },
                [&]() -> int { HIP_TRY(h, hipMemcpyAsync(h->d_window, s_win, sz.win * sizeof(int), hipMemcpyHostToDevice, st)); return CIMPC_OK; },
                [&] { return rekey_in(h); });
            if (rc != CIMPC_OK) return rc;
        }
    }
    if (q_ref) {
        h->st.unlatch();
        auto up = [&](double* dst, double* stg, const double* src, size_t n) -> hipError_t {
            if (n == 0) return hipSuccess;
            if (src) std::memcpy(stg, src, n * sizeof(double)); else std::memset(stg, 0, n * sizeof(double));
            return hipMemcpyAsync(dst, stg, n * sizeof(double), hipMemcpyHostToDevice, st);
        };
        HIP_TRY(h, up(h->S.ref.q, s_q, q_ref, sz.q));
        HIP_TRY(h, up(h->S.ref.u, s_u, u_ref, sz.u));
        HIP_TRY(h, up(h->S.ref.w, s_w, w_ref, sz.w));
        if (gamma_ref) HIP_TRY(h, up(h->S.ref.g, s_g, gamma_ref, sz.g));
        if (b_ref) HIP_TRY(h, up(h->S.ref.b, s_b, b_ref, sz.b));
        HIP_TRY(h, up(h->S.ref.th, s_th, theta_ref, sz.th));
        h->st.reference_replaced();
    }
    if (alt) {
        std::memcpy(s_alt, alt, sz.alt * sizeof(double));
        HIP_TRY(h, hipMemcpyAsync(h->d_alt, s_alt, sz.alt * sizeof(double), hipMemcpyHostToDevice, st));
        h->st.altitude_set();
    }
    int rc = cimpc_newton_solve(h, q0, q1, warm_start, u1, newton_iters, r_norm);
    if (rc != CIMPC_OK) return rc;
    if (q || u || gamma || b || nu_dual) {
        auto down = [&](double* stg, const double* src, double* dst, size_t n) -> hipError_t {
            return (dst && n) ? hipMemcpyAsync(stg, src, n * sizeof(double), hipMemcpyDeviceToHost, st) : hipSuccess;
        };
        HIP_TRY(h, down(s_q, h->S.traj.q, q, sz.q));
        HIP_TRY(h, down(s_u, h->S.traj.u, u, sz.u));
        HIP_TRY(h, down(s_g, h->S.traj.g, gamma, sz.g));
        HIP_TRY(h, down(s_b, h->S.traj.b, b, sz.b));
        HIP_TRY(h, down(s_th, h->S.nu, nu_dual, sz.nu));
        HIP_TRY(h, hipStreamSynchronize(st));
        if (q) std::memcpy(q, s_q, sz.q * sizeof(double));
        if (u) std::memcpy(u, s_u, sz.u * sizeof(double));
        if (gamma && sz.g) std::memcpy(gamma, s_g, sz.g * sizeof(double));
        if (b && sz.b) std::memcpy(b, s_b, sz.b * sizeof(double));
        if (nu_dual) std::memcpy(nu_dual, s_th, sz.nu * sizeof(double));
    }
    return CIMPC_OK;
}

int cimpc_get_trajectory(cimpc_handle h, double* q, double* u, double* gamma, double* b, double* nu_dual) {
    if (!h) return CIMPC_ERR_INVALID;
    const HorizonSizes n = horizon_sizes(h->dm, h->nth, h->nd);
    HIP_TRY(h, hipSetDevice(h->device));
    HIP_TRY(h, hipStreamSynchronize(h->stream));
    if (q) HIP_TRY(h, hipMemcpy(q, h->S.traj.q, n.q * sizeof(double), hipMemcpyDeviceToHost));
    if (u) HIP_TRY(h, hipMemcpy(u, h->S.traj.u, n.u * sizeof(double), hipMemcpyDeviceToHost));
    if (gamma) HIP_TRY(h, hipMemcpy(gamma, h->S.traj.g, n.g * sizeof(double), hipMemcpyDeviceToHost));
    if (b) HIP_TRY(h, hipMemcpy(b, h->S.traj.b, n.b * sizeof(double), hipMemcpyDeviceToHost));
    if (nu_dual) HIP_TRY(h, hipMemcpy(nu_dual, h->S.nu, n.nu * sizeof(double), hipMemcpyDeviceToHost));
    return CIMPC_OK;
}

int cimpc_get_newton_info(cimpc_handle h, int* newton_iters, double* r_norm, double* u1) {
    if (!h) return CIMPC_ERR_INVALID;
    const cimpc_dims& d = h->dm;
    const size_t B = d.B;
    HIP_TRY(h, hipSetDevice(h->device));
    HIP_TRY(h, hipStreamSynchronize(h->stream));
    if (newton_iters) HIP_TRY(h, hipMemcpy(newton_iters, h->S.newton_l, B * sizeof(int), hipMemcpyDeviceToHost));
    if (r_norm) {
        HIP_TRY(h, hipMemcpy(r_norm, h->S.r_norm, B * sizeof(double), hipMemcpyDeviceToHost));
        for (size_t b = 0; b < B; ++b) r_norm[b] /= (double)h->N;
    }
    if (u1)
        HIP_TRY(h, hipMemcpy2D(u1, d.nu * sizeof(double), h->S.traj.u, (size_t)d.H * d.nu * sizeof(double),
                               d.nu * sizeof(double), B, hipMemcpyDeviceToHost));
    return CIMPC_OK;
}

int cimpc_get_rollout_counters(cimpc_handle h, int* sweeps, int* ip_iters, int* ip_failures) {
    if (!h) return CIMPC_ERR_INVALID;
    const size_t B = h->dm.B;
    HIP_TRY(h, hipSetDevice(h->device));
    HIP_TRY(h, hipStreamSynchronize(h->stream));
    if (sweeps) HIP_TRY(h, hipMemcpy(sweeps, h->S.ro_sweeps, B * sizeof(int), hipMemcpyDeviceToHost));
    if (ip_iters) HIP_TRY(h, hipMemcpy(ip_iters, h->S.ro_ip_iters, B * sizeof(int), hipMemcpyDeviceToHost));
    if (ip_failures) HIP_TRY(h, hipMemcpy(ip_failures, h->S.ro_ip_fail, B * sizeof(int), hipMemcpyDeviceToHost));
    return CIMPC_OK;
}

static GaitDev gait_dev(cimpc_ctx* h) {
    return GaitDev{h->g_q, h->g_u, h->g_w, h->g_g, h->g_b, h->g_th, h->g_stride, h->g_phase, h->dm.H_ref};
}

int cimpc_set_gait(cimpc_handle h, const double* q, const double* u, const double* w, const double* gamma,
                   const double* b, const double* theta, const double* stride, const int* phase) {
    if (!h || !q || !u || !theta || !stride) return fail(h, CIMPC_ERR_INVALID, "q, u, theta, stride are required");
    h->st.unlatch();
    const cimpc_dims& d = h->dm;
    const size_t K = d.H_ref, B = d.B;
    if (d.H > d.H_ref) return fail(h, CIMPC_ERR_INVALID, "H_mpc must not exceed H_ref");
    if (phase) for (size_t i = 0; i < B; ++i) if (phase[i] < 0) return fail(h, CIMPC_ERR_INVALID, "negative phase");
    HIP_TRY(h, hipSetDevice(h->device));
    if (int dp = drain_pending(h); dp != CIMPC_OK) return dp;
    if (!h->g_q) {
        if (dev_alloc(h, &h->g_q, (K + 2) * d.nq) != CIMPC_OK || dev_alloc(h, &h->g_u, K * d.nu) != CIMPC_OK ||
            dev_alloc(h, &h->g_w, K * d.nw) != CIMPC_OK || dev_alloc(h, &h->g_g, K * d.nc) != CIMPC_OK ||
            dev_alloc(h, &h->g_b, K * d.nb) != CIMPC_OK || dev_alloc(h, &h->g_th, K * h->nth) != CIMPC_OK ||
            dev_alloc(h, &h->g_stride, d.nq) != CIMPC_OK || dev_alloc(h, &h->g_phase, B) != CIMPC_OK)
            return CIMPC_ERR_HIP;
    }
    HIP_TRY(h, hipMemcpy(h->g_q, q, (K + 2) * d.nq * sizeof(double), hipMemcpyHostToDevice));
    HIP_TRY(h, hipMemcpy(h->g_u, u, K * d.nu * sizeof(double), hipMemcpyHostToDevice));
    auto opt = [&](double* dst, const double* src, size_t n) {
        return src ? hipMemcpy(dst, src, n * sizeof(double), hipMemcpyHostToDevice) : hipMemset(dst, 0, n * sizeof(double));
    };
    HIP_TRY(h, opt(h->g_w, w, K * d.nw));
    HIP_TRY(h, opt(h->g_g, gamma, K * d.nc));
    HIP_TRY(h, opt(h->g_b, b, K * d.nb));
    HIP_TRY(h, hipStreamSynchronize(nullptr));
    HIP_TRY(h, hipMemcpy(h->g_th, theta, K * h->nth * sizeof(double), hipMemcpyHostToDevice));
    HIP_TRY(h, hipMemcpy(h->g_stride, stride, d.nq * sizeof(double), hipMemcpyHostToDevice));
    if (phase) HIP_TRY(h, hipMemcpy(h->g_phase, phase, B * sizeof(int), hipMemcpyHostToDevice));
    else { HIP_TRY(h, hipMemset(h->g_phase, 0, B * sizeof(int))); HIP_TRY(h, hipStreamSynchronize(nullptr)); }
    int rc = window_move(h->st, WindowHome::Device, nullptr, 0, [&] { return rekey_out(h); },
        [&] { int rg = launch_gait_window(h->S, gait_dev(h), h->d_window, 0, h->stream); return rg == CIMPC_OK ? CIMPC_OK : fail(h, rg, "gait window launch failed"); },
        [&] { return then_sync(h, rekey_in(h)); });
    if (rc != CIMPC_OK) return rc;
    h->st.gait_installed();
    return CIMPC_OK;
}

int cimpc_mpc_advance(cimpc_handle h, const double* stride) {
    if (!h || !stride) return fail(h, CIMPC_ERR_INVALID, "null argument");
    if (int rc = refuse(h, h->st.advance_refusal()); rc != CIMPC_OK) return rc;
    h->st.unlatch();
    HIP_TRY(h, hipSetDevice(h->device));
    if (int dp = drain_pending(h); dp != CIMPC_OK) return dp;
    double* st_pin = h->h_qin + 2 * (size_t)h->dm.B * h->dm.nq;
    std::memcpy(st_pin, stride, (size_t)h->dm.nq * sizeof(double));
    auto launched = [&](int rc) { return rc == CIMPC_OK ? CIMPC_OK : fail(h, rc, "mpc_advance launch failed"); };
    if (h->st.advances_by_gait()) {
        int rc = window_move(h->st, WindowHome::Device, nullptr, 0,
            [&]() -> int { HIP_TRY(h, hipMemcpyAsync(h->g_stride, st_pin, (size_t)h->dm.nq * sizeof(double), hipMemcpyHostToDevice, h->stream)); return rekey_out(h); },
            [&] { return launched(launch_gait_window(h->S, gait_dev(h), h->d_window, 1, h->stream)); },
            [&] { return rekey_in(h); });
        if (rc == CIMPC_OK) h->st.advance_queued();
        return rc;
    }
    return window_move(h->st, WindowHome::Device, nullptr, 0,
        [&]() -> int { HIP_TRY(h, hipMemcpyAsync(h->d_q0, stride, (size_t)h->dm.nq * sizeof(double), hipMemcpyHostToDevice, h->stream)); return rekey_out(h); },
        [&] { return launched(launch_mpc_advance(h->S, h->d_window, h->d_q0, h->dm.H_ref, h->stream)); },
        [&] { return then_sync(h, rekey_in(h)); });
}

int cimpc_set_gains(cimpc_handle h, const double* K) {
    if (!h) return CIMPC_ERR_INVALID;
    HIP_TRY(h, hipSetDevice(h->device));
    if (int dp = drain_pending(h); dp != CIMPC_OK) return dp;
    h->st.gains_changing();
    if (!K) { h->st.gains_cleared(); return CIMPC_OK; }
    const cimpc_dims& d = h->dm;
    const size_t nk = (size_t)d.nu * 2 * d.nq;
    if (!h->d_gK && dev_alloc(h, &h->d_gK, (size_t)d.H_ref * nk) != CIMPC_OK) return CIMPC_ERR_HIP;
    if (!h->d_glatch && dev_alloc(h, &h->d_glatch, (size_t)d.B * gain_latch_doubles(d.nq, d.nu)) != CIMPC_OK) return CIMPC_ERR_HIP;
    if (!h->d_gio && dev_alloc(h, &h->d_gio, (size_t)d.B * (2 * d.nq + d.nu)) != CIMPC_OK) return CIMPC_ERR_HIP;
    HIP_TRY(h, hipStreamSynchronize(h->stream));
    HIP_TRY(h, hipMemcpy(h->d_gK, K, (size_t)d.H_ref * nk * sizeof(double), hipMemcpyHostToDevice));
    h->st.gains_replaced();
    return CIMPC_OK;
}

int cimpc_gain_latch(cimpc_handle h) {
    if (!h) return CIMPC_ERR_INVALID;
    if (int rc = refuse(h, h->st.latch_refusal()); rc != CIMPC_OK) return rc;
    HIP_TRY(h, hipSetDevice(h->device));
    if (int dp = drain_pending(h); dp != CIMPC_OK) return dp;
    const cimpc_dims& d = h->dm;
    if (!gain_latch_launch(d.B, d.H, d.nq, d.nu, h->d_window, h->S.traj.u, h->S.ref.q, h->d_gK, h->d_glatch, h->stream))
        return fail(h, CIMPC_ERR_HIP, "gain latch launch failed");
    HIP_TRY(h, hipStreamSynchronize(h->stream));
    h->st.latched();
    return CIMPC_OK;
}

int cimpc_gain_feedback(cimpc_handle h, const double* q_prev, const double* q_cur, double n_sample, double* u) {
    if (!h || !q_prev || !q_cur || !u) return fail(h, CIMPC_ERR_INVALID, "null argument");
    if (!std::isfinite(n_sample) || n_sample <= 0.0) return fail(h, CIMPC_ERR_INVALID, "n_sample must be finite and positive");
    if (int rc = refuse(h, h->st.feedback_refusal()); rc != CIMPC_OK) return rc;
    HIP_TRY(h, hipSetDevice(h->device));
    const cimpc_dims& d = h->dm;
    const size_t nqB = (size_t)d.B * d.nq, nuB = (size_t)d.B * d.nu;
    double* dq = h->d_gio;
    HIP_TRY(h, hipMemcpyAsync(dq, q_prev, nqB * sizeof(double), hipMemcpyHostToDevice, h->stream));
    HIP_TRY(h, hipMemcpyAsync(dq + nqB, q_cur, nqB * sizeof(double), hipMemcpyHostToDevice, h->stream));
    if (!gain_feedback_launch(d.B, d.nq, d.nu, h->d_glatch, dq, dq + nqB, n_sample, dq + 2 * nqB, h->stream))
        return fail(h, CIMPC_ERR_HIP, "gain feedback launch failed");
    HIP_TRY(h, hipMemcpyAsync(u, dq + 2 * nqB, nuB * sizeof(double), hipMemcpyDeviceToHost, h->stream));
    HIP_TRY(h, hipStreamSynchronize(h->stream));
    return CIMPC_OK;
}

int cimpc_get_reference(cimpc_handle h, double* q_ref, double* u_ref, double* w_ref, double* gamma_ref,
                        double* b_ref, double* theta_ref, int* window) {
    if (!h) return CIMPC_ERR_INVALID;
    const HorizonSizes n = horizon_sizes(h->dm, h->nth, h->nd);
    HIP_TRY(h, hipSetDevice(h->device));
    HIP_TRY(h, hipStreamSynchronize(h->stream));
    if (q_ref) HIP_TRY(h, hipMemcpy(q_ref, h->S.ref.q, n.q * sizeof(double), hipMemcpyDeviceToHost));
    if (u_ref) HIP_TRY(h, hipMemcpy(u_ref, h->S.ref.u, n.u * sizeof(double), hipMemcpyDeviceToHost));
    if (w_ref) HIP_TRY(h, hipMemcpy(w_ref, h->S.ref.w, n.w * sizeof(double), hipMemcpyDeviceToHost));
    if (gamma_ref) HIP_TRY(h, hipMemcpy(gamma_ref, h->S.ref.g, n.g * sizeof(double), hipMemcpyDeviceToHost));
    if (b_ref) HIP_TRY(h, hipMemcpy(b_ref, h->S.ref.b, n.b * sizeof(double), hipMemcpyDeviceToHost));
    if (theta_ref) HIP_TRY(h, hipMemcpy(theta_ref, h->S.ref.th, n.th * sizeof(double), hipMemcpyDeviceToHost));
    if (window) {
        HIP_TRY(h, hipMemcpy(window, h->d_window, n.win * sizeof(int), hipMemcpyDeviceToHost));
        for (size_t k = 0; k < n.win; ++k) window[k] += 1;
    }
    return CIMPC_OK;
}

int cimpc_get_newton_log(cimpc_handle h, double* log, int max_entries) {
    if (!h || !log || max_entries <= 0) return CIMPC_ERR_INVALID;
    const size_t B = h->dm.B;
    const int n = std::min(max_entries, NLOG);
    HIP_TRY(h, hipSetDevice(h->device));
    HIP_TRY(h, hipStreamSynchronize(h->stream));
    HIP_TRY(h, hipMemcpy2D(log, (size_t)max_entries * 4 * sizeof(double), h->S.nlog, (size_t)NLOG * 4 * sizeof(double),
                           (size_t)n * 4 * sizeof(double), B, hipMemcpyDeviceToHost));
    return CIMPC_OK;
}

int cimpc_get_kkt_twisted(cimpc_handle h, long long* n) {
    if (!h || !n) return CIMPC_ERR_INVALID;
    *n = h->n_kkt_twisted;
    return CIMPC_OK;
}

int cimpc_get_kkt_twisted_fallbacks(cimpc_handle h, long long* n) {
    if (!h || !n) return CIMPC_ERR_INVALID;
    note_tw_fallbacks(h);
    *n = h->n_kkt_tw_fallbacks;
    return CIMPC_OK;
}

int cimpc_debug_set_tw_spins(cimpc_handle h, int spins) {
    if (!h) return CIMPC_ERR_INVALID;
    h->S.kkt_tw_spins = spins > 0 ? spins : KKT_TW_SPINS;
    return CIMPC_OK;
}

int cimpc_get_kkt_fallbacks(cimpc_handle h, long long* n) {
    if (!h || !n) return CIMPC_ERR_INVALID;
    *n = 0;
    if (!h->d_mix_nfb) return CIMPC_OK;
    int v = 0;
    HIP_TRY(h, hipSetDevice(h->device));
    HIP_TRY(h, hipStreamSynchronize(h->stream));
    HIP_TRY(h, hipMemcpy(&v, h->d_mix_nfb, sizeof(int), hipMemcpyDeviceToHost));
    *n = v;
    return CIMPC_OK;
}

#if defined(CIMPC_KKT_PROF) || defined(CIMPC_KKT_TWPROF)
int cimpc_debug_read_stats(cimpc_handle h, long long* out, int n) {
    if (!h || !out || n > std::max(h->dm.B * 4, 64)) return CIMPC_ERR_INVALID;
    HIP_TRY(h, hipMemcpy(out, h->S.stats, (size_t)n * sizeof(long long), hipMemcpyDeviceToHost));
    return CIMPC_OK;
}
#endif

#ifdef CIMPC_DEBUG_STATS
int cimpc_debug_dump_stats(cimpc_handle h, long long* out, unsigned long long* addr8) {
    if (!h || !out || !addr8) return CIMPC_ERR_INVALID;
    HIP_TRY(h, hipMemcpy(out, h->S.stats, (size_t)h->dm.B * 4 * sizeof(long long), hipMemcpyDeviceToHost));
    const void* a[8] = {h->S.kkt_list, h->S.slot_list, h->S.counters, h->S.stats, h->S.ro_sweeps, h->S.ro_ip_iters, h->S.ro_ip_fail, h->S.nlog};
    for (int k = 0; k < 8; ++k) addr8[k] = (unsigned long long)a[k];
    return CIMPC_OK;
}
#endif

int cimpc_get_stats(cimpc_handle h, cimpc_stats* s) {
    if (!h || !s) return CIMPC_ERR_INVALID;
    *s = h->last_stats;
    return CIMPC_OK;
}

int cimpc_profile_enable(cimpc_handle h, int on) {
    if (!h) return CIMPC_ERR_INVALID;
    prof_collect(h);
    h->prof_on = on == 2 ? 2 : (on != 0 ? 1 : 0);
    return CIMPC_OK;
}

int cimpc_profile_reset(cimpc_handle h) {
    if (!h) return CIMPC_ERR_INVALID;
    prof_collect(h);
    for (int c = 0; c < PC_COUNT; ++c) { h->prof_ms[c] = 0.0; h->prof_n[c] = 0; }
    h->prof_ip_problems = 0;
    h->prof_async_problems = 0;
    h->prof_kkt_systems = 0;
    return CIMPC_OK;
}

int cimpc_profile_read(cimpc_handle h, cimpc_profile* p) {
    if (!h || !p) return CIMPC_ERR_INVALID;
    prof_collect(h);
    p->ip_sweep_ms = h->prof_ms[PC_IP]; p->ip_sweep_launches = h->prof_n[PC_IP];
    p->ip_sweep_problems = h->prof_ip_problems;
    p->kkt_ms = h->prof_ms[PC_KKT]; p->kkt_launches = h->prof_n[PC_KKT]; p->kkt_systems = h->prof_kkt_systems;
    p->resid_ms = h->prof_ms[PC_RESID]; p->resid_launches = h->prof_n[PC_RESID];
    p->other_ms = h->prof_ms[PC_OTHER]; p->other_launches = h->prof_n[PC_OTHER];
    p->async_ms = h->prof_ms[PC_ASYNC]; p->async_launches = h->prof_n[PC_ASYNC]; p->async_problems = h->prof_async_problems;
    return CIMPC_OK;
}

int cimpc_query_sizes(cimpc_handle h, int* table_doubles, int* N_kkt) {
    if (!h) return CIMPC_ERR_INVALID;
    if (table_doubles) *table_doubles = h->ki.tab_size;
    if (N_kkt) *N_kkt = h->N;
    return CIMPC_OK;
}

}

#ifdef CIMPC_UBENCH
extern "C" const double* cimpc_debug_table_ptr(cimpc_handle h) { return h ? h->d_tab : nullptr; }
#endif
```

### contactimplicitmpc/jl_amd/csrc/newton_kernels.hip

```cpp
#include <cstdlib>
#ifdef CIMPC_KKT_PROF
#define CIMPC_KKT_WPROF
#endif
#include "newton_impl.h"
#include "model_table.h"

namespace cimpc {

__global__ __launch_bounds__(256) void reset_kernel(NewtonDev S, const double* q0,
                                                    const double* q1, int warm) {
    const cimpc_dims& m = S.dm;
    const int b = blockIdx.x + S.b0, tid = threadIdx.x, nt = blockDim.x;
    const int H = m.H;
    const size_t oq = (size_t)b * (H + 2) * m.nq;
    const size_t sb0 = (size_t)b * CS;
    if (!warm) {
        for (int k = tid; k < H * S.nd; k += nt) {
            S.nu[(size_t)b * H * S.nd + k] = 0.0;
        }
        copy_n(S.traj.q + oq, S.ref.q + oq, (H + 2) * m.nq, tid, nt);
        copy_n(S.traj.u + (size_t)b * H * m.nu, S.ref.u + (size_t)b * H * m.nu, H * m.nu, tid, nt);
        copy_n(S.traj.w + (size_t)b * H * m.nw, S.ref.w + (size_t)b * H * m.nw, H * m.nw, tid, nt);
        copy_n(S.traj.g + (size_t)b * H * m.nc, S.ref.g + (size_t)b * H * m.nc, H * m.nc, tid, nt);
        copy_n(S.traj.b + (size_t)b * H * m.nb, S.ref.b + (size_t)b * H * m.nb, H * m.nb, tid, nt);
        copy_n(S.traj.th + (size_t)b * H * S.nth, S.ref.th + (size_t)b * H * S.nth, H * S.nth, tid, nt);
    }
    __syncthreads();
    for (int k = tid; k < m.nq; k += nt) {
        S.traj.q[oq + k] = q0[(size_t)b * m.nq + k];
        S.traj.q[oq + m.nq + k] = q1[(size_t)b * m.nq + k];
    }
    __syncthreads();
    theta_update(S, S.traj, b, 0, tid, nt);
    if (H > 1) theta_update(S, S.traj, b, 1, tid, nt);
    __syncthreads();
    copy_n(S.cand.q + sb0 * (H + 2) * m.nq, S.traj.q + oq, (H + 2) * m.nq, tid, nt);
    copy_n(S.cand.u + sb0 * H * m.nu, S.traj.u + (size_t)b * H * m.nu, H * m.nu, tid, nt);
    copy_n(S.cand.w + sb0 * H * m.nw, S.traj.w + (size_t)b * H * m.nw, H * m.nw, tid, nt);
    copy_n(S.cand.g + sb0 * H * m.nc, S.traj.g + (size_t)b * H * m.nc, H * m.nc, tid, nt);
    copy_n(S.cand.b + sb0 * H * m.nb, S.traj.b + (size_t)b * H * m.nb, H * m.nb, tid, nt);
    copy_n(S.cand.th + sb0 * H * S.nth, S.traj.th + (size_t)b * H * S.nth, H * S.nth, tid, nt);
    copy_n(S.nu_cand + sb0 * H * S.nd, S.nu + (size_t)b * H * S.nd, H * S.nd, tid, nt);
    for (int c = 1; c < CS; ++c)
        copy_n(S.cand.w + (sb0 + c) * H * m.nw, S.traj.w + (size_t)b * H * m.nw, H * m.nw, tid, nt);
    if (tid == 0) {
        S.beta[b] = S.beta_init;
        S.stage[b] = STAGE_INIT;
        for (int c = 1; c < CS; ++c) S.need_sweep[sb0 + c] = 0;
        S.cur_slot[b] = 0;
        S.newton_l[b] = 0;
        S.alpha[b] = 1.0;
        S.ls_iter[b] = 0;
        S.r_norm[b] = 0.0;
        S.ro_sweeps[b] = 0;
        S.ro_ip_iters[b] = 0;
        S.ro_ip_fail[b] = 0;
    }
    for (int k = tid; k < CS * H; k += nt) S.pflag[sb0 * H + k] = 0;
    __syncthreads();
    if (S.A.on) enqueue_eval_async<BlockSync>(S, sb0, 0, 1, b, tid, nt);
    else enqueue_eval(S, sb0, b, S.WQ.par, tid, nt, b - S.b0);
}

template <int NQ, int NU>
static int launch_kkt_t(const NewtonDev& S, const KktArgs& K, KktForm f, bool f32, hipStream_t s) {
    if (f == KktForm::PerRollout) {
        if (NQ > 24 || NU > 24 || S.dm.H > kkt_max_h<NQ, NU>()) return CIMPC_ERR_INVALID;
        const size_t lds = (size_t)kkt_lds_doubles<NQ, NU, 1>() * sizeof(double);
        static LdsOptIn optin, optin32;
        if (f32) return launch_lds(optin32, kkt_kernel<NQ, NU, true>, dim3(S.nb_launch), dim3(64), lds, s, S, K);
        return launch_lds(optin, kkt_kernel<NQ, NU>, dim3(S.nb_launch), dim3(64), lds, s, S, K);
    }
    if (f != KktForm::Scalar || f32) return CIMPC_ERR_INVALID;
    constexpr int LD = ((NQ > NU ? NQ : NU) + 3) & ~3;
    static LdsOptIn optin;
    return launch_lds(optin, kkt_kernel_scalar<NQ, NU>, dim3(S.nb_launch), dim3(64), (size_t)(KKT_TILES * LD * LD + 10 * LD) * sizeof(double), s, S, K);
}

template <int NQ, int NU>
static int launch_kkt_list_t(const NewtonDev& S, const KktArgs& K, KktForm f, const int* list, int n, const int* n_dev, hipStream_t s) {
    if constexpr (NQ <= 24 && NU <= 24) {
        if (S.dm.H > kkt_max_h<NQ, NU>()) return CIMPC_ERR_INVALID;
        if constexpr (kkt_tld<NQ, NU>() == 16) if (f == KktForm::Duo) {
            static LdsOptIn optin;
            return launch_lds(optin, kkt_kernel_duo<NQ, NU>, dim3(n), dim3(128), (size_t)(kkt_duo_slice_doubles(1) + kkt_duo_slice_doubles(2)) * sizeof(double),
                              s, KktTwArgs{S, K, list, n, n_dev});
        }
        if (f == KktForm::Twisted) {
            static LdsOptIn optin;
            return launch_lds(optin, kkt_kernel_twisted<NQ, NU>, dim3(2 * n), dim3(192), (size_t)kkt_tw_lds_doubles<NQ, NU>() * sizeof(double), s,
                              KktTwArgs{S, K, list, n, n_dev});
        }
        if (f == KktForm::Pipelined && list != nullptr) {
            static LdsOptIn optin;
            return launch_lds(optin, kkt_kernel_pipe<NQ, NU>, dim3(n), dim3(192), (size_t)kkt_lds_doubles<NQ, NU, 3>() * sizeof(double), s, S, K, list, n, n_dev);
        }
        if (f == KktForm::Packed && list != nullptr) {
            constexpr int PACK = kkt_pack<NQ, NU>();
            static LdsOptIn optin;
            return launch_lds(optin, kkt_kernel_packed<NQ, NU>, dim3((n + PACK - 1) / PACK), dim3(64 * PACK), (size_t)PACK * kkt_lds_doubles<NQ, NU, 1>() * sizeof(double),
                              s, S, K, list, n, n_dev);
        }
    }
    return CIMPC_ERR_INVALID;
}
static int launch_kkt_condensed(const NewtonDev& S, const KktArgs& K, KktForm f, bool f32, const int* list, int n, const int* n_dev, hipStream_t s) {
    if (S.dm.mode != CIMPC_MODE_CONFIGURATION) return CIMPC_ERR_INVALID;
    const bool rollout = f == KktForm::PerRollout || f == KktForm::Scalar;
    if (n_dev != nullptr) n = S.dm.B;
    if (n <= 0) return CIMPC_OK;
    const int nq = S.dm.nq, nu = S.dm.nu;
#define X(name, q, u, w, c, b, a) if (nq == q && nu == u) return rollout ? launch_kkt_t<q, u>(S, K, f, f32, s) : f32 ? CIMPC_ERR_INVALID : launch_kkt_list_t<q, u>(S, K, f, list, n, n_dev, s);
    CIMPC_MODEL_TABLE(X)
#undef X
    return CIMPC_ERR_INVALID;
}

__device__ __forceinline__ double kkt_apply_row(const NewtonDev& S, const double* dzb, const double* x, double rho, int e) {
    const int H = S.dm.H, nq = S.dm.nq, nu = S.dm.nu, nr = nq + nu, nd = nq, blk = (2 * nq + nu) * nd;
    const double* nuv = x + (size_t)H * nr;
    if (e >= H * nr) {
        const int i = (e - H * nr) / nd, k = (e - H * nr) - i * nd;
        const double* dz = dzb + (size_t)i * blk;
        double s = -x[(size_t)i * nr + nu + k] - rho * nuv[(size_t)i * nd + k];
        for (int c = 0; c < nu; ++c) s = fma(dz[(size_t)(2 * nq + c) * nd + k], x[(size_t)i * nr + c], s);
        if (i >= 1) for (int c = 0; c < nq; ++c) s = fma(dz[(size_t)(nq + c) * nd + k], x[(size_t)(i - 1) * nr + nu + c], s);
        if (i >= 2) for (int c = 0; c < nq; ++c) s = fma(dz[(size_t)c * nd + k], x[(size_t)(i - 2) * nr + nu + c], s);
        return s;
    }
    const int i = e / nr, c = e - i * nr;
    double s = 0.0;
    if (c < nu) {
        const double* Rm = S.R + (size_t)i * nu * nu;
        for (int k = 0; k < nu; ++k) s = fma(Rm[c + k * nu], x[(size_t)i * nr + k], s);
        const double* A0 = dzb + (size_t)i * blk + (size_t)(2 * nq + c) * nd;
        for (int k = 0; k < nd; ++k) s = fma(A0[k], nuv[(size_t)i * nd + k], s);
        return s;
    }
    const int cq = c - nu;
    const double* Qm = S.Q + (size_t)i * nq * nq;
    for (int k = 0; k < nq; ++k) s = fma(Qm[cq + k * nq], x[(size_t)i * nr + nu + k], s);
    s -= nuv[(size_t)i * nd + cq];
    if (i + 1 < H) {
        const double* A1 = dzb + (size_t)(i + 1) * blk + (size_t)(nq + cq) * nd;
        for (int k = 0; k < nd; ++k) s = fma(A1[k], nuv[(size_t)(i + 1) * nd + k], s);
    }
    if (i + 2 < H) {
        const double* A2 = dzb + (size_t)(i + 2) * blk + (size_t)cq * nd;
        for (int k = 0; k < nd; ++k) s = fma(A2[k], nuv[(size_t)(i + 2) * nd + k], s);
    }
    return s;
}
struct MixArgs {
    int* flag;
    double* corr;
    double* res;
    double tol;
    int last;
    int* n_fallback;
};
__global__ __launch_bounds__(256) void kkt_mixed_init_kernel(NewtonDev S, KktArgs K, int* flag) {
    const int b = blockIdx.x * 256 + threadIdx.x + S.b0;
    if (b < S.b0 + S.nb_launch) flag[b] = (K.stage == nullptr || K.stage[b] == STAGE_KKT) ? 1 : 0;
}
__global__ __launch_bounds__(256) void kkt_mixed_check_kernel(NewtonDev S, KktArgs K, MixArgs M) {
    const int b = blockIdx.x + S.b0, tid = threadIdx.x, nt = blockDim.x;
    if (M.flag[b] == 0) return;
    __shared__ double red[2 * 256];
    const int N = S.N, H = S.dm.H;
    double* D = K.delta + (size_t)b * N;
    const double* r = K.r + (size_t)b * N;
    if (M.corr != nullptr) {
        const double* c = M.corr + (size_t)b * N;
        for (int e = tid; e < N; e += nt) D[e] += c[e];
        __syncthreads();
    }
    const double beta = K.beta ? K.beta[b] : K.beta_scalar;
    const double rho = (double)H * beta * S.kappa;
    const double* dzb = kkt_dz(S, K, b, H, S.nths, S.nd);
    double* res = M.res + (size_t)b * N;
    double mr = 0.0, mres = 0.0;
    for (int e = tid; e < N; e += nt) {
        const double v = r[e] - kkt_apply_row(S, dzb, D, rho, e);
        res[e] = v;
        mr = fmax(mr, fabs(r[e]));
        mres = (v == v) ? fmax(mres, fabs(v)) : HUGE_VAL;
    }
    red[tid] = mr; red[256 + tid] = mres;
    __syncthreads();
    for (int st = nt / 2; st > 0; st >>= 1) {
        if (tid < st) { red[tid] = fmax(red[tid], red[tid + st]); red[256 + tid] = fmax(red[256 + tid], red[256 + tid + st]); }
        __syncthreads();
    }
    const bool ok = red[256] <= M.tol * fmax(1.0, red[0]);
    __syncthreads();
    if (ok) {
        if (tid == 0) M.flag[b] = 0;
        if (K.finish) {
            __threadfence_block();
            start_line_search<BlockSync>(S, b, 1, tid, nt);
        }
    } else if (M.last && tid == 0 && M.n_fallback != nullptr) {
        atomicAdd(M.n_fallback, 1);
    }
}
size_t kkt_mixed_workspace_doubles(const NewtonDev& S) { return 2 * (size_t)S.dm.B * S.N + (size_t)S.dm.B; }
bool kkt_mixed_available(const NewtonDev& S) {
    return S.dm.mode == CIMPC_MODE_CONFIGURATION && S.V == nullptr && S.dm.nq <= 24 && S.dm.nu <= 24 && S.dm.H <= 96;
}
static int launch_kkt_mixed(const NewtonDev& S, const KktArgs& K0, double* ws, int* n_fallback, hipStream_t s) {
    const size_t BN = (size_t)S.dm.B * S.N;
    double* corr = ws; double* res = ws + BN;
    int* flag = reinterpret_cast<int*>(ws + 2 * BN);
    hipLaunchKernelGGL(kkt_mixed_init_kernel, dim3((S.nb_launch + 255) / 256), dim3(256), 0, s, S, K0, flag);
    KktArgs P = K0; P.finish = 0; P.only_flag = flag;
    int rc = launch_kkt_condensed(S, P, KktForm::PerRollout, true, nullptr, S.nb_launch, nullptr, s);
    if (rc != CIMPC_OK) return rc;
    constexpr int CORRECTIONS = 4;
    for (int k = 0; k <= CORRECTIONS; ++k) {
        MixArgs M{flag, k == 0 ? nullptr : corr, res, 1.0e-9, k == CORRECTIONS ? 1 : 0, n_fallback};
        hipLaunchKernelGGL(kkt_mixed_check_kernel, dim3(S.nb_launch), dim3(256), 0, s, S, K0, M);
        if (k == CORRECTIONS) break;
        KktArgs Pk = P; Pk.r = res; Pk.delta = corr;
        rc = launch_kkt_condensed(S, Pk, KktForm::PerRollout, true, nullptr, S.nb_launch, nullptr, s);
        if (rc != CIMPC_OK) return rc;
    }
    KktArgs F = K0; F.only_flag = flag;
    rc = launch_kkt_condensed(S, F, KktForm::PerRollout, false, nullptr, S.nb_launch, nullptr, s);
    if (rc != CIMPC_OK) return rc;
    return hipGetLastError() == hipSuccess ? CIMPC_OK : CIMPC_ERR_HIP;
}

#ifdef CIMPC_RESID_PROF
extern "C" int cimpc_debug_resid_prof(unsigned long long* out32) {
    unsigned long long z[64] = {0};
    if (hipMemcpyFromSymbol(out32, HIP_SYMBOL(cimpc::g_resid_prof), sizeof(z)) != hipSuccess) return -1;
    return hipMemcpyToSymbol(HIP_SYMBOL(cimpc::g_resid_prof), z, sizeof(z)) == hipSuccess ? 0 : -1;
}
#endif
__global__ __launch_bounds__(64) void enqueue_all_kernel(NewtonDev S) {
    const int b = blockIdx.x + S.b0;
    enqueue_eval(S, (size_t)b * CS, b, S.WQ.par, threadIdx.x, 64, b - S.b0);
    if (threadIdx.x == 0) S.cur_slot[b] = 0;
    for (int k = threadIdx.x; k < S.dm.H; k += 64) S.pflag[(size_t)b * CS * S.dm.H + k] = 0;
}
int launch_enqueue_all(const NewtonDev& S, hipStream_t s) {
    hipLaunchKernelGGL(enqueue_all_kernel, dim3(S.nb_launch), dim3(64), 0, s, S);
    return hipGetLastError() == hipSuccess ? CIMPC_OK : CIMPC_ERR_HIP;
}
__global__ __launch_bounds__(64) void async_handoff_kernel(NewtonDev S, IpQueues LQ) {
    const int i = blockIdx.x, tid = threadIdx.x;
    if (i < S.WQ.K) {
        const int n = *qcount(LQ, LQ.par, i);
        const int* src = LQ.items + ((size_t)LQ.par * LQ.K + i) * LQ.cap;
        int* dst = S.WQ.items + (size_t)i * S.WQ.cap;
        for (int k = tid; k < n; k += 64) dst[k] = src[k];
        if (tid == 0) *qcount(S.WQ, 0, i) = n;
    }
    if (i < S.dm.B && tid == 0) {
        const int b = i, stage = S.stage[b];
        if (stage == STAGE_DONE) {
            atomicAdd(S.A.n_done, 1);
        } else if (stage == STAGE_KKT) {
            push_kkt_job(S.A, b);
        } else {
            const size_t sb0 = (size_t)b * CS;
            int n = 0;
            for (int c = 0; c < CS; ++c) n += (S.need_sweep[sb0 + c] != 0 && S.WQ.done_count[sb0 + c] < S.dm.H);
            S.A.evals_left[b] = n;
        }
    }
}
int launch_async_handoff(const NewtonDev& S, const IpQueues& LQ, hipStream_t s) {
    const int grid = S.dm.B > S.WQ.K ? S.dm.B : S.WQ.K;
    hipLaunchKernelGGL(async_handoff_kernel, dim3(grid), dim3(64), 0, s, S, LQ);
    return hipGetLastError() == hipSuccess ? CIMPC_OK : CIMPC_ERR_HIP;
}
__global__ __launch_bounds__(64) void mpc_advance_kernel(NewtonDev S, int* window, const double* stride, int H_ref) {
    const cimpc_dims& m = S.dm;
    const int b = blockIdx.x, c = threadIdx.x, H = m.H, nq = m.nq, nth = S.nth;
    auto rot = [&](double* a, int rows, int n) {
        if (c >= n) return;
        const double first = a[c];
        for (int t = 0; t + 1 < rows; ++t) a[(size_t)t * n + c] = a[(size_t)(t + 1) * n + c];
        a[(size_t)(rows - 1) * n + c] = first;
    };
    double* q = S.ref.q + (size_t)b * (H + 2) * nq;
    double* th = S.ref.th + (size_t)b * H * nth;
    rot(q, H + 2, nq);
    rot(S.ref.u + (size_t)b * H * m.nu, H, m.nu);
    rot(S.ref.w + (size_t)b * H * m.nw, H, m.nw);
    rot(S.ref.g + (size_t)b * H * m.nc, H, m.nc);
    rot(S.ref.b + (size_t)b * H * m.nb, H, m.nb);
    rot(th, H, nth);
    __syncthreads();
    if (c < nq) {
        q[(size_t)H * nq + c] = q[c] + stride[c];
        q[(size_t)(H + 1) * nq + c] = q[nq + c] + stride[c];
    }
    __syncthreads();
    if (c < nq) {
        for (int tau = H - 2; tau <= H; ++tau) {
            if (tau < 1) continue;
            th[(size_t)(tau - 1) * nth + c] = q[(size_t)(tau - 1) * nq + c];
            th[(size_t)(tau - 1) * nth + nq + c] = q[(size_t)tau * nq + c];
        }
    }
    for (int i = c; i < H + 2; i += 64) {
        int* w = window + (size_t)b * (H + 2) + i;
        *w = (*w + 1) % H_ref;
    }
}
__global__ __launch_bounds__(128) void gait_window_kernel(NewtonDev S, GaitDev G, int* window, int advance) {
    const cimpc_dims& m = S.dm;
    const int b = blockIdx.x, tid = threadIdx.x, nt = blockDim.x, H = m.H, nq = m.nq, nth = S.nth, Hr = G.H_ref;
    const int k = G.phase[b] + advance;
    __syncthreads();
    if (tid == 0) G.phase[b] = k;
    double* q = S.ref.q + (size_t)b * (H + 2) * nq;
    double* th = S.ref.th + (size_t)b * H * nth;
    for (int e = tid; e < (H + 2) * nq; e += nt) {
        const int i = e / nq, c = e - i * nq, a = k + i;
        const int lap = a >= 1 ? (a - 1) / Hr : 0, j = a >= 1 ? (a - 1) - lap * Hr + 1 : 0;
        q[e] = (k == 0 && a == Hr + 1) ? G.q[(size_t)a * nq + c]
                                       : (lap ? G.q[(size_t)j * nq + c] + (double)lap * G.stride[c] : G.q[(size_t)j * nq + c]);
    }
    auto rows = [&](double* dst, const double* src, int n) {
        for (int e = tid; e < H * n; e += nt) {
            const int i = e / n, c = e - i * n;
            dst[e] = src[(size_t)((k + i) % Hr) * n + c];
        }
    };
    rows(S.ref.u + (size_t)b * H * m.nu, G.u, m.nu);
    rows(S.ref.w + (size_t)b * H * m.nw, G.w, m.nw);
    rows(S.ref.g + (size_t)b * H * m.nc, G.g, m.nc);
    rows(S.ref.b + (size_t)b * H * m.nb, G.b, m.nb);
    rows(th, G.th, nth);
    __syncthreads();
    for (int e = tid; e < H * 2 * nq; e += nt) {
        const int i = e / (2 * nq), c = e - i * 2 * nq;
        th[(size_t)i * nth + c] = q[(size_t)i * nq + c];
    }
    for (int i = tid; i < H + 2; i += nt) window[(size_t)b * (H + 2) + i] = (k + i) % Hr;
}
int launch_gait_window(const NewtonDev& S, const GaitDev& G, int* window, int advance, hipStream_t s) {
    hipLaunchKernelGGL(gait_window_kernel, dim3(S.dm.B), dim3(128), 0, s, S, G, window, advance);
    return hipGetLastError() == hipSuccess ? CIMPC_OK : CIMPC_ERR_HIP;
}
int launch_mpc_advance(const NewtonDev& S, int* window, const double* stride, int H_ref, hipStream_t s) {
    hipLaunchKernelGGL(mpc_advance_kernel, dim3(S.dm.B), dim3(64), 0, s, S, window, stride, H_ref);
    return hipGetLastError() == hipSuccess ? CIMPC_OK : CIMPC_ERR_HIP;
}
__global__ __launch_bounds__(128) void dz_rekey_kernel(double* step_base, size_t stride_b, size_t stride_i, double* knot,
                                                       const int* window, int H, int K, int blk, int dir) {
    const int b = (int)blockIdx.x / H, i = (int)blockIdx.x - b * H;
    const int* w = window + (size_t)b * (H + 2);
    const int t = w[i];
    if (dir == 0)
        for (int j = i + 1; j < H; ++j) if (w[j] == t) return;
    double* st = step_base + (size_t)b * stride_b + (size_t)i * stride_i;
    double* kn = knot + ((size_t)b * K + t) * (size_t)blk;
    const double* src = dir == 0 ? st : kn;
    double* dst = dir == 0 ? kn : st;
    for (int e = (int)threadIdx.x; e < blk; e += (int)blockDim.x) dst[e] = src[e];
}
int launch_dz_rekey(const NewtonDev& S, double* knot, const int* window, int which, int dir, hipStream_t s) {
    const size_t blk = (size_t)S.nths * S.nd, H = S.dm.H;
    double* base = which == 0 ? S.dz_good : S.dz;
    const size_t stride_b = which == 0 ? H * blk : (size_t)CS * H * blk;
    hipLaunchKernelGGL(dz_rekey_kernel, dim3(S.dm.B * S.dm.H), dim3(128), 0, s, base, stride_b, blk, knot, window, S.dm.H, S.dm.H_ref, (int)blk, dir);
    return hipGetLastError() == hipSuccess ? CIMPC_OK : CIMPC_ERR_HIP;
}
int launch_reset(const NewtonDev& S, const double* q0, const double* q1, int warm, hipStream_t s) {
    hipLaunchKernelGGL(reset_kernel, dim3(S.nb_launch), dim3(256), 0, s, S, q0, q1, warm);
    return hipGetLastError() == hipSuccess ? CIMPC_OK : CIMPC_ERR_HIP;
}
template <int NQ, int NU, bool CF>
static int launch_resid_m(const NewtonDev& S, hipStream_t s, int n_slots, int phase) {
    const size_t lds2 = (size_t)2 * CIMPC_RESID_THREADS * sizeof(double);
    if (n_slots == -1) {
        const size_t lds1 = (size_t)(CS * 256 + S.N) * sizeof(double);
        if (lds1 <= 64 * 1024) {
            if (phase == 1) return CIMPC_OK;
            hipLaunchKernelGGL((resid_decide_kernel<NQ, NU, CF, true>), dim3(S.nb_launch), dim3(CIMPC_RESID_THREADS), lds1, s, S);
            return hipGetLastError() == hipSuccess ? CIMPC_OK : CIMPC_ERR_HIP;
        }
    }
    const int* list = (n_slots >= 0 && S.slot_list != nullptr) ? S.slot_list + (size_t)S.WQ.par * S.dm.B * CS : nullptr;
    const int grid = list != nullptr ? n_slots : S.nb_launch * CS;
    const size_t lds = (size_t)(256 + (S.N <= SLOT_ABS_MAX ? S.N : 0)) * sizeof(double);
    if (grid > 0 && phase != 2) hipLaunchKernelGGL((resid_slot_kernel<NQ, NU, CF>), dim3(grid), dim3(CIMPC_SLOT_THREADS), lds, s, S, list);
    if (phase != 1) hipLaunchKernelGGL((resid_decide_kernel<NQ, NU, CF, false>), dim3(S.nb_launch), dim3(CIMPC_RESID_THREADS), lds2, s, S);
    return hipGetLastError() == hipSuccess ? CIMPC_OK : CIMPC_ERR_HIP;
}
template <int NQ, int NU>
static int launch_resid_t(const NewtonDev& S, hipStream_t s, int n_slots, int phase) {
    return S.dm.mode == CIMPC_MODE_CONFIGURATIONFORCE ? launch_resid_m<NQ, NU, true>(S, s, n_slots, phase) : launch_resid_m<NQ, NU, false>(S, s, n_slots, phase);
}
__global__ __launch_bounds__(256) void solve_finish_kernel(NewtonDev S, double* out) {
    __shared__ double red[RESULT_SUMS][256];
    const int tid = threadIdx.x, B = S.dm.B, H = S.dm.H, nu = S.dm.nu;
    double acc[RESULT_SUMS] = {0.0, 0.0, 0.0, 0.0, 0.0};
    for (int b = tid; b < B; b += 256) {
        for (int k = 0; k < RESULT_STATS; ++k) acc[k] += (double)S.stats[(size_t)b * 4 + k];
        acc[RESULT_NEWTON_SUM] += (double)S.newton_l[b];
        double* o = out + result_u1(b, nu);
        for (int k = 0; k < nu; ++k) o[k] = S.traj.u[(size_t)b * H * nu + k];
        o[record_iters(nu)] = (double)S.newton_l[b];
        o[record_r_norm(nu)] = S.r_norm[b];
    }
    for (int k = 0; k < RESULT_SUMS; ++k) red[k][tid] = acc[k];
    __syncthreads();
    for (int st = 128; st > 0; st >>= 1) {
        if (tid < st) for (int k = 0; k < RESULT_SUMS; ++k) red[k][tid] += red[k][tid + st];
        __syncthreads();
    }
    if (tid < RESULT_SUMS) out[tid] = red[tid][0];
}
__global__ __launch_bounds__(256) void dz_commit_kernel(NewtonDev S) {
    const int b = blockIdx.x, i = blockIdx.y, tid = threadIdx.x, H = S.dm.H;
    const int blk = S.nths * S.nd;
    const int s_ = S.good_src[(size_t)b * H + i];
    if (s_ < 0) return;
    double* good = S.dz_good + ((size_t)b * H + i) * blk;
    const double* slot = S.dz + (((size_t)b * CS + s_) * H + i) * blk;
    for (int e = tid; e < blk; e += 256) good[e] = slot[e];
    __syncthreads();
    if (tid == 0) S.good_src[(size_t)b * H + i] = -1;
}
int launch_dz_commit(const NewtonDev& S, hipStream_t s) {
    if (S.good_src == nullptr) return CIMPC_OK;
    hipLaunchKernelGGL(dz_commit_kernel, dim3(S.dm.B, S.dm.H), dim3(256), 0, s, S);
    return hipGetLastError() == hipSuccess ? CIMPC_OK : CIMPC_ERR_HIP;
}
bool kkt_mfma_available(const NewtonDev& S) {
    const int nq = S.dm.nq, nu = S.dm.nu;
    if (S.dm.mode != CIMPC_MODE_CONFIGURATION || nq > 24 || nu > 24) return false;
#define X(name, q, u, w, c, b, a) if (nq == q && nu == u) return S.dm.H <= kkt_max_h<q, u>();
    CIMPC_MODEL_TABLE(X)
#undef X
    return false;
}
bool kkt_packed_available(const NewtonDev& S) {
    return S.dm.mode == CIMPC_MODE_CONFIGURATION && S.kkt_list != nullptr && S.dm.nq <= 24 && S.dm.nu <= 24 && S.dm.H <= 96 && kkt_condensed_available(S);
}
int launch_solve_finish(const NewtonDev& S, double* out, hipStream_t s) {
    hipLaunchKernelGGL(solve_finish_kernel, dim3(1), dim3(256), 0, s, S, out);
    return hipGetLastError() == hipSuccess ? CIMPC_OK : CIMPC_ERR_HIP;
}
__global__ void queue_recycle_kernel(IpQueues Q, int par) {
    const int k = (int)(blockIdx.x * blockDim.x + threadIdx.x);
    if (k < Q.K) { *qcount(Q, par, k) = 0; *qhead(Q, k) = 0; }
}
int launch_queue_recycle(const IpQueues& Q, int par, hipStream_t s) {
    hipLaunchKernelGGL(queue_recycle_kernel, dim3((Q.K + 255) / 256), dim3(256), 0, s, Q, par);
    return hipGetLastError() == hipSuccess ? CIMPC_OK : CIMPC_ERR_HIP;
}
int launch_resid_decide(const NewtonDev& S, hipStream_t s, int n_slots, int phase) {
    const int nq = S.dm.nq, nu = S.dm.nu;
#define X(name, q, u, w, c, b, a) if (nq == q && nu == u) return launch_resid_t<q, u>(S, s, n_slots, phase);
    CIMPC_MODEL_TABLE(X)
#undef X
    return launch_resid_t<0, 0>(S, s, n_slots, phase);
}
struct CfReduce { double* dzq; double* r2; double* d2; };
__global__ __launch_bounds__(256) void cf_reduce_pre_kernel(NewtonDev S, KktArgs K, CfReduce W) {
    const int b = blockIdx.x + S.b0, tid = threadIdx.x, nt = blockDim.x;
    if (K.stage != nullptr && K.stage[b] != STAGE_KKT) return;
    const int nq = S.dm.nq, nu = S.dm.nu, ny = S.dm.nc + S.dm.nb, H = S.dm.H, nr = S.nr, nd = S.nd, nths = S.nths;
    const int nr2 = nu + nq, N2 = H * (nr2 + nq);
    const double* dz = kkt_dz(S, K, b, H, nths, nd);
    const double* r = K.r + (size_t)b * S.N;
    double* dzq = W.dzq + (size_t)b * H * nths * nq;
    double* r2 = W.r2 + (size_t)b * N2;
    for (int e = tid; e < H * nths * nq; e += nt) {
        const int ic = e / nq, rr = e - ic * nq;
        dzq[e] = dz[(size_t)ic * nd + rr];
    }
    auto dot_y = [&](int i, int c) {
        const double* col = dz + ((size_t)i * nths + c) * nd + nq;
        const double* ry = r + (size_t)i * nr + nu;
        double acc = 0.0;
        for (int k = 0; k < ny; ++k) acc = fma(col[k], ry[k], acc);
        return acc;
    };
    for (int e = tid; e < H * nr2; e += nt) {
        const int j = e / nr2, k = e - j * nr2;
        double v;
        if (k < nu) v = r[(size_t)j * nr + k] + dot_y(j, 2 * nq + k);
        else {
            const int cq = k - nu;
            v = r[(size_t)j * nr + nu + ny + cq];
            if (j + 1 < H) v += dot_y(j + 1, nq + cq);
            if (j + 2 < H) v += dot_y(j + 2, cq);
        }
        r2[e] = v;
    }
    for (int e = tid; e < H * nq; e += nt) {
        const int i = e / nq, k = e - i * nq;
        r2[(size_t)H * nr2 + e] = r[(size_t)H * nr + (size_t)i * nd + k];
    }
}

__global__ __launch_bounds__(256) void cf_reduce_post_kernel(NewtonDev S, KktArgs K, CfReduce W) {
    const int b = blockIdx.x + S.b0, tid = threadIdx.x, nt = blockDim.x;
    if (K.stage != nullptr && K.stage[b] != STAGE_KKT) return;
    const int nq = S.dm.nq, nu = S.dm.nu, nc = S.dm.nc, nbb = S.dm.nb, ny = nc + nbb, H = S.dm.H, nr = S.nr, nd = S.nd, nths = S.nths;
    const int nr2 = nu + nq, N2 = H * (nr2 + nq);
    const double* dz = kkt_dz(S, K, b, H, nths, nd);
    const double* r = K.r + (size_t)b * S.N;
    const double* d2 = W.d2 + (size_t)b * N2;
    double* D = K.delta + (size_t)b * S.N;
    const double beta = K.beta ? K.beta[b] : K.beta_scalar;
    const double rho = (double)H * beta * S.kappa;
    for (int e = tid; e < H * nr2; e += nt) {
        const int j = e / nr2, k = e - j * nr2;
        D[(size_t)j * nr + (k < nu ? k : ny + k)] = d2[e];
    }
    for (int e = tid; e < H * nq; e += nt) {
        const int i = e / nq, k = e - i * nq;
        D[(size_t)H * nr + (size_t)i * nd + k] = d2[(size_t)H * nr2 + e];
    }
    for (int e = tid; e < H * ny; e += nt) {
        const int i = e / ny, k = e - i * ny;
        double s = 0.0;
        for (int c = 0; c < nths; ++c) {
            double x;
            if (c < nq) x = i >= 2 ? d2[(size_t)(i - 2) * nr2 + nu + c] : 0.0;
            else if (c < 2 * nq) x = i >= 1 ? d2[(size_t)(i - 1) * nr2 + nu + (c - nq)] : 0.0;
            else x = d2[(size_t)i * nr2 + (c - 2 * nq)];
            s = fma(dz[((size_t)i * nths + c) * nd + nq + k], x, s);
        }
        D[(size_t)i * nr + nu + k] = s + rho * r[(size_t)i * nr + nu + k] - r[(size_t)H * nr + (size_t)i * nd + nq + k];
    }
    __syncthreads();
    for (int e = tid; e < H * ny; e += nt) {
        const int i = e / ny, k = e - i * ny;
        double g = 0.0;
        if (k < nc) { for (int c = 0; c < nc; ++c) g = fma(S.Cg[(size_t)i * nc * nc + (size_t)c * nc + k], D[(size_t)i * nr + nu + c], g); }
        else { const int kb = k - nc; for (int c = 0; c < nbb; ++c) g = fma(S.Cb[(size_t)i * nbb * nbb + (size_t)c * nbb + kb], D[(size_t)i * nr + nu + nc + c], g); }
        D[(size_t)H * nr + (size_t)i * nd + nq + k] = g - r[(size_t)i * nr + nu + k];
    }
    __syncthreads();
    if (K.finish) {
        if (S.kkt_tw_flags != nullptr) {
            const int* fl = S.kkt_tw_flags + (size_t)b * KKT_TW_FLAGS;
            if (aload(fl + TW_TIMED_OUT) == S.kkt_tw_epoch || aload(fl + KKT_BAND_TW_FLAG0 + TW_TIMED_OUT) == S.kkt_tw_epoch) {
                if (tid == 0) {
                    const int pos = atomicAdd(round_counter(S.counters, RC_KKT), 1);
                    if (S.kkt_list != nullptr && pos < S.dm.B) S.kkt_list[(size_t)S.WQ.par * S.dm.B + pos] = b;
                }
                return;
            }
        }
        __threadfence_block();
        start_line_search<BlockSync>(S, b, 1, tid, nt);
    }
}

NewtonDev cf_shadow(const NewtonDev& S) {
    NewtonDev S2 = S;
    S2.dm.mode = CIMPC_MODE_CONFIGURATION;
    S2.nd = S.dm.nq; S2.nr = S.dm.nu + S.dm.nq; S2.N = S.dm.H * (S.dm.nu + 2 * S.dm.nq);
    S2.Cg = nullptr; S2.Cb = nullptr;
    return S2;
}
size_t cf_reduce_doubles(const NewtonDev& S) {
    return (size_t)S.dm.B * ((size_t)S.dm.H * S.nths * S.dm.nq + 2 * (size_t)S.dm.H * (S.dm.nu + 2 * S.dm.nq));
}
static int launch_kkt_cf_reduced(const NewtonDev& S, const KktArgs& K, bool banded, KktForm f, const KktWorkspace& W, hipStream_t s) {
    const size_t B = S.dm.B, n_dz = (size_t)S.dm.H * S.nths * S.dm.nq, N2 = (size_t)S.dm.H * (S.dm.nu + 2 * S.dm.nq);
    CfReduce R{W.cf, W.cf + B * n_dz, W.cf + B * n_dz + B * N2};
    hipLaunchKernelGGL(cf_reduce_pre_kernel, dim3(S.nb_launch), dim3(256), 0, s, S, K, R);
    const NewtonDev S2 = cf_shadow(S);
    const KktArgs K2{R.r2, R.d2, K.beta, K.beta_scalar, K.stage, 0, R.dzq};
    const KktForm f2 = kkt_mfma_available(S2) ? KktForm::PerRollout : KktForm::Scalar;
    const int rc = banded ? launch_kkt_dense(S2, K2, f, W.dense, s) : launch_kkt_condensed(S2, K2, f2, false, nullptr, S.nb_launch, nullptr, s);
    if (rc != CIMPC_OK) return rc;
    hipLaunchKernelGGL(cf_reduce_post_kernel, dim3(S.nb_launch), dim3(256), 0, s, S, K, R);
    return hipGetLastError() == hipSuccess ? CIMPC_OK : CIMPC_ERR_HIP;
}
bool kkt_cf_reduce_available(const NewtonDev& S) {
    return S.dm.mode == CIMPC_MODE_CONFIGURATIONFORCE && (S.V != nullptr ? kkt_banded_available(cf_shadow(S)) : kkt_condensed_available(S));
}

bool kkt_twisted_available(const NewtonDev& S) {
    return kkt_packed_available(S) && S.dm.H >= KKT_TW_MIN_H && S.kkt_tw_xch != nullptr;
}
bool kkt_duo_available(const NewtonDev& S) {
    return S.dm.nq <= 16 && S.dm.nu <= 16 && kkt_twisted_available(S);
}
bool kkt_condensed_available(const NewtonDev& S) {
    return model_has_nqnu(S.dm.nq, S.dm.nu);
}

int launch_kkt_stage(const NewtonDev& S, const KktArgs& K, KktBackend be, KktForm f, const int* list, int n, const int* n_dev,
                     const KktWorkspace& W, hipStream_t s) {
    const bool banded = f == KktForm::BandedOneEnded || f == KktForm::BandedTwisted;
    switch (be) {
    case KktBackend::Condensed: return launch_kkt_condensed(S, K, f, false, list, n, n_dev, s);
    case KktBackend::CondensedMixed: return f == KktForm::PerRollout ? launch_kkt_mixed(S, K, W.mix, W.mix_nfb, s) : CIMPC_ERR_INVALID;
    case KktBackend::Banded: return banded ? launch_kkt_dense(S, K, f, W.dense, s) : CIMPC_ERR_INVALID;
    case KktBackend::DenseLu: return f == KktForm::Dense ? launch_kkt_dense(S, K, f, W.dense, s) : CIMPC_ERR_INVALID;
    case KktBackend::CfCondensed: return f == KktForm::PerRollout ? launch_kkt_cf_reduced(S, K, false, f, W, s) : CIMPC_ERR_INVALID;
    case KktBackend::CfBanded: return banded ? launch_kkt_cf_reduced(S, K, true, f, W, s) : CIMPC_ERR_INVALID;
    }
    return CIMPC_ERR_INVALID;
}

}
```

### contactimplicitmpc/jl_amd/csrc/newton_state.h

```cpp
#pragma once
#include "cimpc_internal.h"
#include "kkt_plan.h"

namespace cimpc {
constexpr int NLOG = 16;

enum Stage : int { STAGE_DONE = 0, STAGE_INIT = 1, STAGE_LS0 = 2, STAGE_KKT = 3, STAGE_LS1 = 4, STAGE_LS2 = 5, STAGE_LS7 = 6, STAGE_LS3 = 7 };
constexpr int CS = 7;

struct TrajDev {
    double* q;
    double* u;
    double* w;
    double* g;
    double* b;
    double* th;
};

struct NewtonDev {
    cimpc_dims dm;
    int b0;
    int nb_launch;
    int kkt_same_round;
    int nd, nr, nth, nths, N;
    TrajDev traj, cand, ref;
    double* nu;
    double* nu_cand;
    double* d;
    double* dz;
    double* dtn;
    int dtn_ld;
    double* dz_good;
    int* good_src;
    int* ip_status;
    int* ip_iters;
    int* pflag;
    int* cur_slot;
    IpQueues WQ;
    AsyncQ A;
    double* res;
    double* res_cand;
    double* delta;
    double* r_norm;
    double* r_cand;
    double* alpha;
    double* beta;
    int* ls_iter;
    int* newton_l;
    int* stage;
    int* kkt_list;
    int* need_sweep;
    int* slot_list;
    int* counters;
    int* counters_next;
    int* host_flag;
    int round_stamp;
    int band_reduce;
    int band_form;
    long long* stats;
    int* ro_sweeps;
    int* ro_ip_iters;
    int* ro_ip_fail;
    const double* Q;
    const double* R;
    const double* Qinv;
    const double* Rinv;
    const double* Cg;
    const double* Cb;
    const double* V;
    const double* q_target;
    const double* v_target;
    double* kkt_ws;
    double* kkt_tw_xch;
    int* kkt_tw_flags;
    int kkt_tw_epoch;
    int kkt_tw_spins;
    int* kkt_tw_fail;
    int kkt_tw_nb;
    double r_tol, beta_init, kappa;
    int max_iter;
    double* nlog;
    int spec_first;
    int spec_mid;
    int spec_all;
};

bool newton_async_available(const cimpc_dims* dm);
int launch_newton_async(const cimpc_dims* dm, const IpParams& p, const NewtonDev& S, int waves, int grid, hipStream_t s);
int launch_async_handoff(const NewtonDev& S, const IpQueues& lockstep_next, hipStream_t s);
int launch_mpc_advance(const NewtonDev& S, int* window, const double* stride, int H_ref, hipStream_t s);
struct GaitDev {
    const double *q, *u, *w, *g, *b, *th;
    const double* stride;
    int* phase;
    int H_ref;
};
int launch_gait_window(const NewtonDev& S, const GaitDev& G, int* window, int advance, hipStream_t s);
int launch_reset(const NewtonDev& nd, const double* q0, const double* q1, int warm, hipStream_t s);
int launch_dz_commit(const NewtonDev& nd, hipStream_t s);
int launch_dz_rekey(const NewtonDev& nd, double* knot, const int* window, int which, int dir, hipStream_t s);
int launch_resid_decide(const NewtonDev& nd, hipStream_t s, int n_slots = -1, int phase = 0);
int launch_enqueue_all(const NewtonDev& nd, hipStream_t s);
struct KktArgs {
    const double* r;
    double* delta;
    const double* beta;
    double beta_scalar;
    const int* stage;
    int finish;
    const double* dz_override;
    const int* only_flag;
};
inline KktArgs kkt_newton_args(const NewtonDev& S) { return KktArgs{S.res, S.delta, S.beta, 0.0, S.stage, 1, nullptr, nullptr}; }
inline KktArgs kkt_raw_args(const double* r, double beta, double* delta) { return KktArgs{r, delta, nullptr, beta, nullptr, 0, nullptr, nullptr}; }
struct KktWorkspace { double* dense; double* cf; double* mix; int* mix_nfb; };
int launch_kkt_stage(const NewtonDev& S, const KktArgs& K, KktBackend be, KktForm f, const int* list, int n, const int* n_dev,
                     const KktWorkspace& W, hipStream_t s);
bool kkt_condensed_available(const NewtonDev& nd);
bool kkt_mfma_available(const NewtonDev& nd);
bool kkt_packed_available(const NewtonDev& nd);
bool kkt_twisted_available(const NewtonDev& nd);
bool kkt_duo_available(const NewtonDev& nd);
bool kkt_mixed_available(const NewtonDev& nd);
bool kkt_banded_available(const NewtonDev& S);
bool kkt_banded_twisted_available(const NewtonDev& S);
bool kkt_cf_reduce_available(const NewtonDev& S);
size_t kkt_mixed_workspace_doubles(const NewtonDev& nd);
size_t kkt_dense_workspace_doubles(const NewtonDev& S, bool banded);
size_t cf_reduce_doubles(const NewtonDev& S);
NewtonDev cf_shadow(const NewtonDev& S);
int launch_queue_recycle(const IpQueues& Q, int par, hipStream_t s);
int launch_solve_finish(const NewtonDev& nd, double* out, hipStream_t s);
int launch_kkt_dense(const NewtonDev& S, const KktArgs& K, KktForm f, double* ws, hipStream_t s);

}
```

### contactimplicitmpc/jl_amd/csrc/round_protocol.h

```cpp
#pragma once
#include <stddef.h>

#if defined(__HIPCC__)
#define ROUND_HD __host__ __device__ __forceinline__
#else
#define ROUND_HD inline
#endif

namespace cimpc {

constexpr int QPAD = 32;
constexpr int CPAD = 32;

enum RoundCounter : int {
    RC_SWEEP = 0,
    RC_KKT = 1,
    RC_PARKED = 2,
    RC_DRAINED = 3,
    RC_SLOTS = 4,
    RC_NEW_SLOTS = 5,
    RC_TICKET = 7,
};
constexpr int ROUND_COUNTERS = 8;
constexpr int ROUND_COUNTER_INTS = ROUND_COUNTERS * CPAD;
ROUND_HD constexpr int* round_counter(int* block, int k) { return block + k * CPAD; }
ROUND_HD constexpr int* round_counter_block(int* blocks, int parity) { return blocks + ROUND_COUNTER_INTS * parity; }

enum RingWord : int {
    RING_N_SWEEP = 0,
    RING_N_KKT = 1,
    RING_STAMP = 2,
    RING_ABORT = 3,
    RING_PARKED = 4,
    RING_FINISHED = 5,
    RING_SLOTS = 6,
    RING_NEW_SLOTS = 7,
};
constexpr int RING_SLOT_INTS = 8, RING_SLOTS_COUNT = 2, RING_ALLOC_INTS = 32;
constexpr RingWord RING_PUBLISHED[] = {RING_N_SWEEP, RING_N_KKT, RING_PARKED, RING_SLOTS, RING_NEW_SLOTS, RING_FINISHED, RING_STAMP};
template <class T> ROUND_HD constexpr T* ring_slot(T* ring, long long round) { return ring + RING_SLOT_INTS * (round & 1); }
template <class T> ROUND_HD constexpr T* ring_abort_word(T* ring) { return ring + RING_ABORT; }

struct QueueCtl { size_t count, head, counters, ints; };
constexpr QueueCtl queue_ctl(size_t K) { return {0, 2 * K * QPAD, 3 * K * QPAD, 3 * K * QPAD + 2 * (size_t)ROUND_COUNTER_INTS}; }

constexpr int EPOCH_STRIDE = 16, EPOCH_BUCKETS = 16, EPOCH_WORDS = 2 * EPOCH_BUCKETS + 1;
constexpr int ASYNC_JOB_INTS = 64;
struct AsyncCtl { size_t count, head, jobs, rq_head, n_done, rq_tail, kq_head, kq_tail, epoch, ints; };
constexpr AsyncCtl async_ctl(size_t K) {
    const size_t j = 2 * K * QPAD;
    return {0, K * QPAD, j, j + 0, j + 8, j + 16, j + 32, j + 48, j + ASYNC_JOB_INTS, j + ASYNC_JOB_INTS + EPOCH_WORDS * EPOCH_STRIDE};
}
ROUND_HD constexpr int epoch_bucket(int i) { return i & (EPOCH_BUCKETS - 1); }
ROUND_HD constexpr int epoch_ip(int bucket) { return bucket * EPOCH_STRIDE; }
ROUND_HD constexpr int epoch_job(int bucket) { return (EPOCH_BUCKETS + bucket) * EPOCH_STRIDE; }
ROUND_HD constexpr int epoch_any_job() { return 2 * EPOCH_BUCKETS * EPOCH_STRIDE; }

constexpr int KJOB_SHIFT = 24, KJOB_MASK = (1 << KJOB_SHIFT) - 1;
enum KktJobKind : int {
    KJOB_ONE_ENDED = 0,
    KJOB_TOP = 1,
    KJOB_BOTTOM = 2,
    KJOB_RETRY = 3,
};

enum TwFlag : int {
    TW_TRACES = 0,
    TW_MIDDLE = 1,
    TW_FINISHED = 2,
    TW_TIMED_OUT = 3,
};
constexpr int KKT_BAND_TW_FLAG0 = 4;
constexpr int KKT_TW_FLAGS = 32;
constexpr int KKT_TW_SPINS = 1 << 21;
ROUND_HD constexpr int kkt_tw_xch_doubles(int nd) { return 3 * nd * nd + 4 * nd; }

enum ResultWord : int { RESULT_SWEEPS = 0, RESULT_IP_SOLVES = 1, RESULT_IP_ITERS = 2, RESULT_IP_FAILURES = 3, RESULT_NEWTON_SUM = 4 };
constexpr int RESULT_STATS = 4, RESULT_SUMS = 5, RESULT_HEADER = 8;
ROUND_HD constexpr int result_record(int nu) { return nu + 2; }
ROUND_HD constexpr size_t result_doubles(size_t B, int nu) { return RESULT_HEADER + B * (size_t)result_record(nu); }
ROUND_HD constexpr size_t result_u1(size_t b, int nu) { return RESULT_HEADER + b * (size_t)result_record(nu); }
ROUND_HD constexpr int record_iters(int nu) { return nu; }
ROUND_HD constexpr int record_r_norm(int nu) { return nu + 1; }

}
```

Measured before the change: 74650.

## Trim per-solve edge overhead with mapped results, kernel-side resets and event waits

Adds a default-on lean_edges mode that cuts per-solve host-side operations. The finish kernel now writes results straight into mapped pinned host memory and zeroes the queue/control counters itself, which removes the D2H memcpy and the next solve's memsets. The host spin-waits on a done event instead of synchronizing the stream, and the dz commit is moved after that event so later calls order on a commit event. A lean reset kernel and a handoff-side ip_before reduction replace a stats memset and a host stats read. The change risks ordering bugs between the deferred commit and later operations, and the spin-wait burns a host core.

```diff
diff --git a/contactimplicitmpc/jl_amd/csrc/cimpc_host.cpp b/contactimplicitmpc/jl_amd/csrc/cimpc_host.cpp
--- a/contactimplicitmpc/jl_amd/csrc/cimpc_host.cpp
+++ b/contactimplicitmpc/jl_amd/csrc/cimpc_host.cpp
@@ -39,6 +39,8 @@
     hipStream_t st_kkt = nullptr;
     hipEvent_t ev_join = nullptr;
     hipEvent_t ev_start = nullptr;
+    hipEvent_t ev_done = nullptr;
+    hipEvent_t ev_commit = nullptr;
 };
 
 struct Knobs {
@@ -47,6 +49,7 @@
     double watchdog_s = 30.0;
     bool debug_rounds = false;
     bool generic_static = false;
+    bool lean_edges = true;
     KktPolicy kkt{};
     int kkt_tw_nb = 0;
     int kkt_tw_spins = 0;
@@ -72,7 +75,7 @@
         kkt.kkt_duo = env_int("CIMPC_KKT_DUO", kkt.kkt_duo);
         kkt.kkt_duo_hint = env_int("CIMPC_KKT_DUO_HINT", kkt.kkt_duo_hint);
         kkt.async_kkt_tw = env_int("CIMPC_ASYNC_KKT_TW", kkt.async_kkt_tw);
-        generic_static = env_int("CIMPC_GENERIC_STATIC", generic_static ? 1 : 0) != 0;
+        lean_edges = env_int("CIMPC_LEAN_EDGES", lean_edges ? 1 : 0) != 0;
         sched.sweep_wgs = env_int("CIMPC_SWEEP_WGS", sched.sweep_wgs);
         sched.waves32 = env_int("CIMPC_WAVES32", sched.waves32);
         banded_form = env_int("CIMPC_BANDED_FORM", banded_form);
@@ -108,6 +111,10 @@
     size_t h_stage_doubles = 0;
     double* d_result = nullptr;
     double* h_result = nullptr;
+    double* h_result_dev = nullptr;
+    bool ctl_clean = false;
+    bool commit_pending = false;
+    hipStream_t commit_stream = nullptr;
     double* d_rhs = nullptr;
     double* d_pstate = nullptr;
     long long ip_budget_ticks = 0;
@@ -500,7 +507,8 @@
     if (rc == CIMPC_OK) h->d_q1 = h->d_q0 + B * d.nq;
     A(&h->d_result, result_doubles(B, d.nu));
     if (rc == CIMPC_OK && (hipHostMalloc((void**)&h->h_qin, (2 * B + 1) * d.nq * sizeof(double), hipHostMallocDefault) != hipSuccess ||
-                           hipHostMalloc((void**)&h->h_result, result_doubles(B, d.nu) * sizeof(double), hipHostMallocDefault) != hipSuccess))
+                           hipHostMalloc((void**)&h->h_result, result_doubles(B, d.nu) * sizeof(double), hipHostMallocMapped) != hipSuccess ||
+                           hipHostGetDevicePointer((void**)&h->h_result_dev, h->h_result, 0) != hipSuccess))
         rc = CIMPC_ERR_HIP;
     A(&h->d_rhs, B * h->N);
     NewtonDev& S = h->S;
@@ -528,6 +536,7 @@
     A(&S.counters, ROUND_COUNTER_INTS);
     A(&S.stats, std::max<size_t>(B * 4, 64));
     A(&S.ro_sweeps, B); A(&S.ro_ip_iters, B); A(&S.ro_ip_fail, B); A(&S.nlog, B * NLOG * 4);
+    A(&S.ip_before, 1);
     A(&S.kkt_ws, B * H * (3 * (size_t)h->nd * h->nd + h->nd));
     A(&S.kkt_tw_xch, B * kkt_tw_xch_doubles(h->nd));
     A(&S.kkt_tw_flags, B * KKT_TW_FLAGS);
@@ -578,7 +587,9 @@
         if (hipStreamCreateWithFlags(&r.st, hipStreamNonBlocking) != hipSuccess ||
             hipStreamCreateWithFlags(&r.st_kkt, hipStreamNonBlocking) != hipSuccess ||
             hipEventCreateWithFlags(&r.ev_join, hipEventDisableTiming) != hipSuccess ||
-            hipEventCreateWithFlags(&r.ev_start, hipEventDisableTiming) != hipSuccess) {
+            hipEventCreateWithFlags(&r.ev_start, hipEventDisableTiming) != hipSuccess ||
+            hipEventCreateWithFlags(&r.ev_done, hipEventDisableTiming) != hipSuccess ||
+            hipEventCreateWithFlags(&r.ev_commit, hipEventDisableTiming) != hipSuccess) {
             g_create_error = "stream creation failed"; cimpc_destroy(h); return CIMPC_ERR_HIP;
         }
     }
@@ -590,6 +601,7 @@
     if (!h) return CIMPC_ERR_INVALID;
     (void)hipSetDevice(h->device);
     if (h->stream) (void)hipStreamSynchronize(h->stream);
+    if (h->rs.st) (void)hipStreamSynchronize(h->rs.st);
     for (auto& r : h->prof_recs) { (void)hipEventDestroy(r.a); (void)hipEventDestroy(r.b); }
     for (auto e : h->ev_pool) (void)hipEventDestroy(e);
     for (void* p : h->allocs) (void)hipFree(p);
@@ -606,6 +618,8 @@
         if (r.st_kkt) { (void)hipStreamSynchronize(r.st_kkt); (void)hipStreamDestroy(r.st_kkt); }
         if (r.ev_join) (void)hipEventDestroy(r.ev_join);
         if (r.ev_start) (void)hipEventDestroy(r.ev_start);
+        if (r.ev_done) (void)hipEventDestroy(r.ev_done);
+        if (r.ev_commit) (void)hipEventDestroy(r.ev_commit);
     }
     if (h->own_stream && h->stream) (void)hipStreamDestroy(h->stream);
     delete h;
@@ -815,6 +829,13 @@
     return CIMPC_OK;
 }
 
+static int order_commit(cimpc_ctx* h) {
+    if (!h->commit_pending) return CIMPC_OK;
+    if (h->commit_stream != h->stream) HIP_TRY(h, hipStreamWaitEvent(h->stream, h->rs.ev_commit, 0));
+    h->commit_pending = false;
+    return CIMPC_OK;
+}
+
 static int sync_dz_stores(cimpc_ctx* h, int next_producer) {
     if (!h->st.dz_sync_needed(next_producer)) return CIMPC_OK;
     const size_t row = (size_t)h->dm.H * h->nths * h->nd * sizeof(double), B = h->dm.B;
@@ -829,11 +850,13 @@
 static int rekey_out(cimpc_ctx* h) {
     if (!h->st.rekey_out_needed()) return CIMPC_OK;
     if (!h->d_dz_knot && dev_alloc(h, &h->d_dz_knot, (size_t)h->dm.B * h->dm.H_ref * h->nths * h->nd) != CIMPC_OK) return CIMPC_ERR_HIP;
+    if (int oc = order_commit(h); oc != CIMPC_OK) return oc;
     int rc = launch_dz_rekey(h->S, h->d_dz_knot, h->d_window, h->st.rekey_out_store(), 0, h->stream);
     return rc == CIMPC_OK ? CIMPC_OK : fail(h, rc, "sensitivity archive launch failed");
 }
 static int rekey_in(cimpc_ctx* h) {
     if (!h->st.rekey_in_needed(h->d_dz_knot != nullptr)) return CIMPC_OK;
+    if (int oc = order_commit(h); oc != CIMPC_OK) return oc;
     for (int which = 0; which < 2; ++which) {
         int rc = launch_dz_rekey(h->S, h->d_dz_knot, h->d_window, which, 1, h->stream);
         if (rc != CIMPC_OK) return fail(h, rc, "sensitivity restore launch failed");
@@ -894,8 +917,10 @@
     if (d.mode == CIMPC_MODE_CONFIGURATIONFORCE && (!gamma || !b))
         return fail(h, CIMPC_ERR_INVALID, "gamma and b are required in configurationforce mode");
     HIP_TRY(h, hipSetDevice(h->device));
+    if (int oc = order_commit(h); oc != CIMPC_OK) return oc;
     if (int sy = sync_dz_stores(h, DZ_IMPLICIT); sy != CIMPC_OK) return sy;
     h->st.implicit_dynamics_started();
+    h->ctl_clean = false;
     TrajDev& T = h->S.cand;
     auto up = [&](double* dst, const double* src, size_t row_doubles) {
         return hipMemcpy2DAsync(dst, CS * row_doubles * sizeof(double), src, row_doubles * sizeof(double),
@@ -981,6 +1006,7 @@
     if (!r || !delta) return fail(h, CIMPC_ERR_INVALID, "null argument");
     const size_t n = (size_t)h->dm.B * h->N;
     HIP_TRY(h, hipSetDevice(h->device));
+    if (int oc = order_commit(h); oc != CIMPC_OK) return oc;
     HIP_TRY(h, hipMemcpyAsync(h->d_rhs, r, n * sizeof(double), hipMemcpyHostToDevice, h->stream));
     if ((rc = ensure_kkt_ws(h)) != CIMPC_OK) return rc;
     for (int attempt = 0; attempt < 2; ++attempt) {
@@ -1062,9 +1088,26 @@
 }
 
 int finish_results(cimpc_ctx* h, hipStream_t st) {
-    if (launch_dz_commit(h->S, st) != CIMPC_OK) return fail(h, CIMPC_ERR_HIP, "sensitivity flush launch failed");
-    if (int rf = launch_solve_finish(h->S, h->d_result, st); rf != CIMPC_OK) return fail(h, rf, "result kernel launch failed");
-    HIP_TRY(h, hipMemcpyAsync(h->h_result, h->d_result, result_doubles(h->dm.B, h->dm.nu) * sizeof(double), hipMemcpyDeviceToHost, st));
+    if (!h->kn.lean_edges) {
+        if (launch_dz_commit(h->S, st) != CIMPC_OK) return fail(h, CIMPC_ERR_HIP, "sensitivity flush launch failed");
+        if (int rf = launch_solve_finish(h->S, h->d_result, SolveTidy{}, st); rf != CIMPC_OK) return fail(h, rf, "result kernel launch failed");
+        HIP_TRY(h, hipMemcpyAsync(h->h_result, h->d_result, result_doubles(h->dm.B, h->dm.nu) * sizeof(double), hipMemcpyDeviceToHost, st));
+        return CIMPC_OK;
+    }
+    const SolveTidy tidy{1, h->Q.count, (int)h->ctl_ints, h->a_ctrl, h->a_ctrl ? (int)async_ctl(h->Q.K).ints : 0};
+    if (int rf = launch_solve_finish(h->S, h->h_result_dev, tidy, st); rf != CIMPC_OK) return fail(h, rf, "result kernel launch failed");
+    HIP_TRY(h, hipEventRecord(h->rs.ev_done, st));
+    if (h->S.good_src != nullptr) {
+        if (launch_dz_commit(h->S, st) != CIMPC_OK) return fail(h, CIMPC_ERR_HIP, "sensitivity flush launch failed");
+        HIP_TRY(h, hipEventRecord(h->rs.ev_commit, st));
+        h->commit_pending = true; h->commit_stream = st;
+    }
+    return CIMPC_OK;
+}
+int wait_results(cimpc_ctx* h, hipStream_t st) {
+    if (!h->kn.lean_edges) { HIP_TRY(h, hipStreamSynchronize(st)); return CIMPC_OK; }
+    while (hipEventQuery(h->rs.ev_done) == hipErrorNotReady) {}
+    HIP_TRY(h, hipEventSynchronize(h->rs.ev_done));
     return CIMPC_OK;
 }
 void publish_stats(cimpc_ctx* h, long long rounds) {
@@ -1100,7 +1143,8 @@
         HIP_TRY(h, hipMemsetAsync(h->a_jobs, 0xFF, (h->a_rq_cap + h->a_kq_cap) * sizeof(int), st));
         h->async_dirty = false;
     }
-    HIP_TRY(h, hipMemsetAsync(h->a_ctrl, 0, async_ctl(h->Q.K).ints * sizeof(int), st));
+    const bool lean = h->kn.lean_edges;
+    if (!lean) HIP_TRY(h, hipMemsetAsync(h->a_ctrl, 0, async_ctl(h->Q.K).ints * sizeof(int), st));
     volatile int* abort_word = ring_abort_word((volatile int*)h->h_ring);
     *abort_word = 0;
     NewtonDev Sk = launch_view(h, 0);
@@ -1115,17 +1159,17 @@
                        .B = h->dm.B, .async_tail = h->sched.async_tail, .waves = std::min(h->sched.waves, 4)};
     A.kkt_tw = plan_kkt_stage(h, site) == KktForm::AsyncTwoJob ? 1 : 0;
     S.kkt_tw_epoch += h->nt.max_iter + 2;
-    prof_begin(h, PC_OTHER, st);
-    int rc2 = from_reset ? launch_reset(Sk, run.q0_dev, run.q1_dev, run.warm_start, st) : launch_async_handoff(Sk, LQ, st);
-    prof_end(h, st);
-    if (rc2 != CIMPC_OK) return fail(h, rc2, "reset / hand-off launch failed");
     IpParams p = make_ip_params(h, S.cand, 0, round_counter(h->d_ring, RC_PARKED), nullptr);
     if (S.dtn != nullptr) { p.nu = S.nu_cand; p.dtn = S.dtn; }
     p.Q = Sk.WQ;
     p.iter_cap = h->ip.max_iter + 1;
     p.A = A;
+    prof_begin(h, PC_OTHER, st);
+    int rc2 = from_reset ? launch_reset(Sk, run.q0_dev, run.q1_dev, run.warm_start, lean, st) : launch_async_handoff(Sk, LQ, lean, st);
+    prof_end(h, st);
+    if (rc2 != CIMPC_OK) return fail(h, rc2, "reset / hand-off launch failed");
     long long solved_before = 0;
-    if (h->prof_on && !from_reset) { long long sv[4]; if (int rs = read_stats(h, sv); rs != CIMPC_OK) return rs; solved_before = sv[1]; }
+    if (h->prof_on && !from_reset && !lean) { long long sv[4]; if (int rs = read_stats(h, sv); rs != CIMPC_OK) return rs; solved_before = sv[1]; }
     prof_begin(h, PC_ASYNC, st);
     rc2 = launch_newton_async(&h->dm, p, Sk, std::min(h->sched.waves, 4), from_reset ? h->sched.async_grid : h->sched.tail_grid, st);
     prof_end(h, st);
@@ -1134,16 +1178,20 @@
     const bool budget = has_time_budget(h);
     bool timed_out = false; long long polls = 0;
     const auto tw = std::chrono::steady_clock::now();
-    while (hipStreamQuery(st) == hipErrorNotReady) {
+    while ((lean ? hipEventQuery(h->rs.ev_done) : hipStreamQuery(st)) == hipErrorNotReady) {
         const bool over = budget && over_budget(h, run);
         timed_out = !over && (++polls & 0x3FF) == 0 && std::chrono::duration<double>(std::chrono::steady_clock::now() - tw).count() > h->kn.watchdog_s;
         if (over || timed_out) { *abort_word = 1; h->async_dirty = true; break; }
     }
-    HIP_TRY(h, hipStreamSynchronize(st));
+    if (int wr = wait_results(h, st); wr != CIMPC_OK) return wr;
     note_tw_fallbacks(h);
     if (timed_out) return fail(h, CIMPC_ERR_HIP, "asynchronous solve: watchdog expired (no completion within CIMPC_ASYNC_WATCHDOG_S)");
     if (h->a_dbg) { if (int rd = print_async_debug(h); rd != CIMPC_OK) return rd; }
     publish_stats(h, rounds_before + 1);
+    if (lean) {
+        h->ctl_clean = !h->async_dirty;
+        if (h->prof_on && !from_reset) solved_before = (long long)h->h_result[RESULT_IP_BEFORE];
+    }
     h->prof_ip_problems += solved_before;
     h->prof_async_problems += h->last_stats.ip_solves - solved_before;
     if (from_reset) h->prof_kkt_systems += h->last_stats.newton_iters;
@@ -1198,6 +1246,8 @@
     if (rc != CIMPC_OK) return rc;
     if (!q0_dev || !q1_dev) return fail(h, CIMPC_ERR_INVALID, "null argument");
     HIP_TRY(h, hipSetDevice(h->device));
+    if (h->commit_pending && h->commit_stream == (h->external_stream ? h->stream : h->rs.st)) h->commit_pending = false;
+    else if (int oc = order_commit(h); oc != CIMPC_OK) return oc;
     if (int sy = sync_dz_stores(h, DZ_NEWTON); sy != CIMPC_OK) return sy;
     h->st.solve_started();
     const int B = h->dm.B;
@@ -1210,7 +1260,16 @@
         HIP_TRY(h, hipEventRecord(sb.ev_start, h->stream));
         HIP_TRY(h, hipStreamWaitEvent(sb.st, sb.ev_start, 0));
     }
-    HIP_TRY(h, hipMemsetAsync(h->S.stats, 0, (size_t)B * 4 * sizeof(long long), sb.st));
+    const bool lean = h->kn.lean_edges;
+    if (!lean) HIP_TRY(h, hipMemsetAsync(h->S.stats, 0, (size_t)B * 4 * sizeof(long long), sb.st));
+    else {
+        if (!h->ctl_clean) {
+            HIP_TRY(h, hipMemsetAsync(h->Q.count, 0, h->ctl_ints * sizeof(int), sb.st));
+            if (h->a_ctrl) HIP_TRY(h, hipMemsetAsync(h->a_ctrl, 0, async_ctl(h->Q.K).ints * sizeof(int), sb.st));
+            HIP_TRY(h, hipMemsetAsync(h->S.ip_before, 0, sizeof(long long), sb.st));
+        }
+        h->ctl_clean = false;
+    }
     if ((rc = ensure_kkt_ws(h)) != CIMPC_OK) return rc;
     const SolvePath path = choose_solve_path(h->sched, h->kb);
     if (path == SolvePath::Persistent) return run_async(h, run, true, 0);
@@ -1218,11 +1277,13 @@
     const int round_limit = max_rounds(h->kn.sched, h->nt.max_iter, h->ip.max_iter);
     long long launched = 0, completed = 0;
     const bool ahead = round_ahead(h->sched, h->kb, warm_start != 0, has_time_budget(h));
-    HIP_TRY(h, hipMemsetAsync(h->Q.count, 0, h->ctl_ints * sizeof(int), sb.st));
-    if (run.hybrid) HIP_TRY(h, hipMemsetAsync(h->a_ctrl + async_ctl(h->Q.K).jobs, 0, ASYNC_JOB_INTS * sizeof(int), sb.st));
+    if (!lean) {
+        HIP_TRY(h, hipMemsetAsync(h->Q.count, 0, h->ctl_ints * sizeof(int), sb.st));
+        if (run.hybrid) HIP_TRY(h, hipMemsetAsync(h->a_ctrl + async_ctl(h->Q.K).jobs, 0, ASYNC_JOB_INTS * sizeof(int), sb.st));
+    }
     for (int slot = 0; slot < RING_SLOTS_COUNT; ++slot) ring_slot((volatile int*)h->h_ring, slot)[RING_STAMP] = 0;
     prof_begin(h, PC_OTHER, sb.st);
-    rc = launch_reset(launch_view(h, 0), q0_dev, q1_dev, warm_start, sb.st);
+    rc = launch_reset(launch_view(h, 0), q0_dev, q1_dev, warm_start, lean, sb.st);
     prof_end(h, sb.st);
     if (rc != CIMPC_OK) return fail(h, rc, "reset launch failed");
     while (true) {
@@ -1251,14 +1312,17 @@
         ++completed;
         if ((last.sweep == 0 && last.kkt == 0) || over_budget(h, run)) break;
         if (run.hybrid && hand_over(h->sched, B - last.finished)) {
-            HIP_TRY(h, hipStreamSynchronize(sb.st));
-            HIP_TRY(h, hipStreamSynchronize(sb.st_kkt));
+            if (!lean) {
+                HIP_TRY(h, hipStreamSynchronize(sb.st));
+                HIP_TRY(h, hipStreamSynchronize(sb.st_kkt));
+            }
             return run_async(h, run, false, completed);
         }
     }
-    HIP_TRY(h, hipStreamSynchronize(sb.st_kkt));
+    if (!lean) HIP_TRY(h, hipStreamSynchronize(sb.st_kkt));
     if (int rf = finish_results(h, sb.st); rf != CIMPC_OK) return rf;
-    HIP_TRY(h, hipStreamSynchronize(sb.st));
+    if (int wr = wait_results(h, sb.st); wr != CIMPC_OK) return wr;
+    if (lean) h->ctl_clean = true;
     publish_stats(h, completed);
     h->prof_ip_problems += h->last_stats.ip_solves;
     return CIMPC_OK;
diff --git a/contactimplicitmpc/jl_amd/csrc/newton_kernels.hip b/contactimplicitmpc/jl_amd/csrc/newton_kernels.hip
--- a/contactimplicitmpc/jl_amd/csrc/newton_kernels.hip
+++ b/contactimplicitmpc/jl_amd/csrc/newton_kernels.hip
@@ -1,3 +1,4 @@
+#include <algorithm>
 #include <cstdlib>
 #ifdef CIMPC_KKT_PROF
 #define CIMPC_KKT_WPROF
@@ -62,6 +63,76 @@
     else enqueue_eval(S, sb0, b, S.WQ.par, tid, nt, b - S.b0);
 }
 
+__global__ __launch_bounds__(256) void lean_reset_kernel(NewtonDev S, const double* q0, const double* q1, int warm) {
+    const cimpc_dims& m = S.dm;
+    const int b = blockIdx.x + S.b0, tid = threadIdx.x, nt = blockDim.x;
+    const int H = m.H, nq = m.nq, nu = m.nu, nw = m.nw, nth = S.nth;
+    const size_t oq = (size_t)b * (H + 2) * nq, ob = (size_t)b * H;
+    const size_t sb0 = (size_t)b * CS;
+    const TrajDev& src = warm ? S.traj : S.ref;
+    auto qv = [&](int k) { return k < nq ? q0[(size_t)b * nq + k] : k < 2 * nq ? q1[(size_t)b * nq + (k - nq)] : src.q[oq + k]; };
+    for (int k = tid; k < (H + 2) * nq; k += nt) {
+        const double v = qv(k);
+        if (!warm || k < 2 * nq) S.traj.q[oq + k] = v;
+        S.cand.q[sb0 * (H + 2) * nq + k] = v;
+    }
+    for (int k = tid; k < H * nu; k += nt) {
+        const double v = src.u[ob * nu + k];
+        if (!warm) S.traj.u[ob * nu + k] = v;
+        S.cand.u[sb0 * H * nu + k] = v;
+    }
+    for (int k = tid; k < H * nw; k += nt) {
+        const double v = src.w[ob * nw + k];
+        if (!warm) S.traj.w[ob * nw + k] = v;
+        for (int c = 0; c < CS; ++c) S.cand.w[(sb0 + c) * H * nw + k] = v;
+    }
+    for (int k = tid; k < H * m.nc; k += nt) {
+        const double v = src.g[ob * m.nc + k];
+        if (!warm) S.traj.g[ob * m.nc + k] = v;
+        S.cand.g[sb0 * H * m.nc + k] = v;
+    }
+    for (int k = tid; k < H * m.nb; k += nt) {
+        const double v = src.b[ob * m.nb + k];
+        if (!warm) S.traj.b[ob * m.nb + k] = v;
+        S.cand.b[sb0 * H * m.nb + k] = v;
+    }
+    const int th_rows = H > 1 ? 2 : 1;
+    for (int k = tid; k < H * nth; k += nt) {
+        const int i = k / nth, c = k - i * nth;
+        const bool upd = i < th_rows && c < 2 * nq + nu + nw;
+        double v;
+        if (!upd) v = src.th[ob * nth + k];
+        else if (c < 2 * nq) v = qv(i * nq + c);
+        else if (c < 2 * nq + nu) v = src.u[(ob + i) * nu + (c - 2 * nq)];
+        else v = src.w[(ob + i) * nw + (c - 2 * nq - nu)];
+        if (!warm || upd) S.traj.th[ob * nth + k] = v;
+        S.cand.th[sb0 * H * nth + k] = v;
+    }
+    for (int k = tid; k < H * S.nd; k += nt) {
+        const double v = warm ? S.nu[ob * S.nd + k] : 0.0;
+        if (!warm) S.nu[ob * S.nd + k] = v;
+        S.nu_cand[sb0 * H * S.nd + k] = v;
+    }
+    if (tid < 4) S.stats[(size_t)b * 4 + tid] = 0;
+    if (tid == 0) {
+        S.beta[b] = S.beta_init;
+        S.stage[b] = STAGE_INIT;
+        for (int c = 1; c < CS; ++c) S.need_sweep[sb0 + c] = 0;
+        S.cur_slot[b] = 0;
+        S.newton_l[b] = 0;
+        S.alpha[b] = 1.0;
+        S.ls_iter[b] = 0;
+        S.r_norm[b] = 0.0;
+        S.ro_sweeps[b] = 0;
+        S.ro_ip_iters[b] = 0;
+        S.ro_ip_fail[b] = 0;
+    }
+    for (int k = tid; k < CS * H; k += nt) S.pflag[sb0 * H + k] = 0;
+    __syncthreads();
+    if (S.A.on) enqueue_eval_async<BlockSync>(S, sb0, 0, 1, b, tid, nt);
+    else enqueue_eval(S, sb0, b, S.WQ.par, tid, nt, b - S.b0);
+}
+
 template <int NQ, int NU>
 static int launch_kkt_t(const NewtonDev& S, const KktArgs& K, KktForm f, bool f32, hipStream_t s) {
     if (f == KktForm::PerRollout) {
@@ -248,8 +319,20 @@
     hipLaunchKernelGGL(enqueue_all_kernel, dim3(S.nb_launch), dim3(64), 0, s, S);
     return hipGetLastError() == hipSuccess ? CIMPC_OK : CIMPC_ERR_HIP;
 }
-__global__ __launch_bounds__(64) void async_handoff_kernel(NewtonDev S, IpQueues LQ) {
+__global__ __launch_bounds__(64) void async_handoff_kernel(NewtonDev S, IpQueues LQ, int lean) {
     const int i = blockIdx.x, tid = threadIdx.x;
+    if (lean && i == 0) {
+        __shared__ long long part[64];
+        long long acc = 0;
+        for (int b = tid; b < S.dm.B; b += 64) acc += S.stats[(size_t)b * 4 + 1];
+        part[tid] = acc;
+        __syncthreads();
+        for (int st = 32; st > 0; st >>= 1) {
+            if (tid < st) part[tid] += part[tid + st];
+            __syncthreads();
+        }
+        if (tid == 0) *S.ip_before = part[0];
+    }
     if (i < S.WQ.K) {
         const int n = *qcount(LQ, LQ.par, i);
         const int* src = LQ.items + ((size_t)LQ.par * LQ.K + i) * LQ.cap;
@@ -260,7 +343,7 @@
     if (i < S.dm.B && tid == 0) {
         const int b = i, stage = S.stage[b];
         if (stage == STAGE_DONE) {
-            atomicAdd(S.A.n_done, 1);
+            if (!lean) atomicAdd(S.A.n_done, 1);
         } else if (stage == STAGE_KKT) {
             push_kkt_job(S.A, b);
         } else {
@@ -271,9 +354,9 @@
         }
     }
 }
-int launch_async_handoff(const NewtonDev& S, const IpQueues& LQ, hipStream_t s) {
+int launch_async_handoff(const NewtonDev& S, const IpQueues& LQ, int lean, hipStream_t s) {
     const int grid = S.dm.B > S.WQ.K ? S.dm.B : S.WQ.K;
-    hipLaunchKernelGGL(async_handoff_kernel, dim3(grid), dim3(64), 0, s, S, LQ);
+    hipLaunchKernelGGL(async_handoff_kernel, dim3(grid), dim3(64), 0, s, S, LQ, lean);
     return hipGetLastError() == hipSuccess ? CIMPC_OK : CIMPC_ERR_HIP;
 }
 __global__ __launch_bounds__(64) void mpc_advance_kernel(NewtonDev S, int* window, const double* stride, int H_ref) {
@@ -371,8 +454,9 @@
     hipLaunchKernelGGL(dz_rekey_kernel, dim3(S.dm.B * S.dm.H), dim3(128), 0, s, base, stride_b, blk, knot, window, S.dm.H, S.dm.H_ref, (int)blk, dir);
     return hipGetLastError() == hipSuccess ? CIMPC_OK : CIMPC_ERR_HIP;
 }
-int launch_reset(const NewtonDev& S, const double* q0, const double* q1, int warm, hipStream_t s) {
-    hipLaunchKernelGGL(reset_kernel, dim3(S.nb_launch), dim3(256), 0, s, S, q0, q1, warm);
+int launch_reset(const NewtonDev& S, const double* q0, const double* q1, int warm, int lean, hipStream_t s) {
+    if (lean) hipLaunchKernelGGL(lean_reset_kernel, dim3(S.nb_launch), dim3(256), 0, s, S, q0, q1, warm);
+    else hipLaunchKernelGGL(reset_kernel, dim3(S.nb_launch), dim3(256), 0, s, S, q0, q1, warm);
     return hipGetLastError() == hipSuccess ? CIMPC_OK : CIMPC_ERR_HIP;
 }
 template <int NQ, int NU, bool CF>
@@ -397,17 +481,19 @@
 static int launch_resid_t(const NewtonDev& S, hipStream_t s, int n_slots, int phase) {
     return S.dm.mode == CIMPC_MODE_CONFIGURATIONFORCE ? launch_resid_m<NQ, NU, true>(S, s, n_slots, phase) : launch_resid_m<NQ, NU, false>(S, s, n_slots, phase);
 }
-__global__ __launch_bounds__(256) void solve_finish_kernel(NewtonDev S, double* out) {
+__global__ __launch_bounds__(256) void solve_finish_kernel(NewtonDev S, double* out, SolveTidy T) {
     __shared__ double red[RESULT_SUMS][256];
     const int tid = threadIdx.x, B = S.dm.B, H = S.dm.H, nu = S.dm.nu;
     double acc[RESULT_SUMS] = {0.0, 0.0, 0.0, 0.0, 0.0};
+    const int rec = result_record(nu);
+    for (int e = (int)blockIdx.x * 256 + tid; e < B * rec; e += (int)gridDim.x * 256) {
+        const int b = e / rec, k = e - b * rec;
+        out[RESULT_HEADER + e] = k < nu ? S.traj.u[(size_t)b * H * nu + k] : k == record_iters(nu) ? (double)S.newton_l[b] : S.r_norm[b];
+    }
+    if (blockIdx.x != 0) return;
     for (int b = tid; b < B; b += 256) {
         for (int k = 0; k < RESULT_STATS; ++k) acc[k] += (double)S.stats[(size_t)b * 4 + k];
         acc[RESULT_NEWTON_SUM] += (double)S.newton_l[b];
-        double* o = out + result_u1(b, nu);
-        for (int k = 0; k < nu; ++k) o[k] = S.traj.u[(size_t)b * H * nu + k];
-        o[record_iters(nu)] = (double)S.newton_l[b];
-        o[record_r_norm(nu)] = S.r_norm[b];
     }
     for (int k = 0; k < RESULT_SUMS; ++k) red[k][tid] = acc[k];
     __syncthreads();
@@ -416,6 +502,10 @@
         __syncthreads();
     }
     if (tid < RESULT_SUMS) out[tid] = red[tid][0];
+    if (!T.on) return;
+    if (tid == 0) { out[RESULT_IP_BEFORE] = (double)*S.ip_before; *S.ip_before = 0; }
+    for (int k = tid; k < T.n_ctl; k += 256) T.ctl[k] = 0;
+    for (int k = tid; k < T.n_actl; k += 256) T.actl[k] = 0;
 }
 __global__ __launch_bounds__(256) void dz_commit_kernel(NewtonDev S) {
     const int b = blockIdx.x, i = blockIdx.y, tid = threadIdx.x, H = S.dm.H;
@@ -444,8 +534,9 @@
 bool kkt_packed_available(const NewtonDev& S) {
     return S.dm.mode == CIMPC_MODE_CONFIGURATION && S.kkt_list != nullptr && S.dm.nq <= 24 && S.dm.nu <= 24 && S.dm.H <= 96 && kkt_condensed_available(S);
 }
-int launch_solve_finish(const NewtonDev& S, double* out, hipStream_t s) {
-    hipLaunchKernelGGL(solve_finish_kernel, dim3(1), dim3(256), 0, s, S, out);
+int launch_solve_finish(const NewtonDev& S, double* out, const SolveTidy& T, hipStream_t s) {
+    const int blocks = T.on ? std::max(1, std::min(64, (S.dm.B * result_record(S.dm.nu) + 255) / 256)) : 1;
+    hipLaunchKernelGGL(solve_finish_kernel, dim3(blocks), dim3(256), 0, s, S, out, T);
     return hipGetLastError() == hipSuccess ? CIMPC_OK : CIMPC_ERR_HIP;
 }
 __global__ void queue_recycle_kernel(IpQueues Q, int par) {
diff --git a/contactimplicitmpc/jl_amd/csrc/newton_state.h b/contactimplicitmpc/jl_amd/csrc/newton_state.h
--- a/contactimplicitmpc/jl_amd/csrc/newton_state.h
+++ b/contactimplicitmpc/jl_amd/csrc/newton_state.h
@@ -58,6 +58,7 @@
     int band_reduce;
     int band_form;
     long long* stats;
+    long long* ip_before;
     int* ro_sweeps;
     int* ro_ip_iters;
     int* ro_ip_fail;
@@ -87,7 +88,7 @@
 
 bool newton_async_available(const cimpc_dims* dm);
 int launch_newton_async(const cimpc_dims* dm, const IpParams& p, const NewtonDev& S, int waves, int grid, hipStream_t s);
-int launch_async_handoff(const NewtonDev& S, const IpQueues& lockstep_next, hipStream_t s);
+int launch_async_handoff(const NewtonDev& S, const IpQueues& lockstep_next, int lean, hipStream_t s);
 int launch_mpc_advance(const NewtonDev& S, int* window, const double* stride, int H_ref, hipStream_t s);
 struct GaitDev {
     const double *q, *u, *w, *g, *b, *th;
@@ -96,7 +97,7 @@
     int H_ref;
 };
 int launch_gait_window(const NewtonDev& S, const GaitDev& G, int* window, int advance, hipStream_t s);
-int launch_reset(const NewtonDev& nd, const double* q0, const double* q1, int warm, hipStream_t s);
+int launch_reset(const NewtonDev& nd, const double* q0, const double* q1, int warm, int lean, hipStream_t s);
 int launch_dz_commit(const NewtonDev& nd, hipStream_t s);
 int launch_dz_rekey(const NewtonDev& nd, double* knot, const int* window, int which, int dir, hipStream_t s);
 int launch_resid_decide(const NewtonDev& nd, hipStream_t s, int n_slots = -1, int phase = 0);
@@ -130,7 +131,8 @@
 size_t cf_reduce_doubles(const NewtonDev& S);
 NewtonDev cf_shadow(const NewtonDev& S);
 int launch_queue_recycle(const IpQueues& Q, int par, hipStream_t s);
-int launch_solve_finish(const NewtonDev& nd, double* out, hipStream_t s);
+struct SolveTidy { int on; int* ctl; int n_ctl; int* actl; int n_actl; };
+int launch_solve_finish(const NewtonDev& nd, double* out, const SolveTidy& tidy, hipStream_t s);
 int launch_kkt_dense(const NewtonDev& S, const KktArgs& K, KktForm f, double* ws, hipStream_t s);
 
 }
diff --git a/contactimplicitmpc/jl_amd/csrc/round_protocol.h b/contactimplicitmpc/jl_amd/csrc/round_protocol.h
--- a/contactimplicitmpc/jl_amd/csrc/round_protocol.h
+++ b/contactimplicitmpc/jl_amd/csrc/round_protocol.h
@@ -75,7 +75,8 @@
 constexpr int KKT_TW_SPINS = 1 << 21;
 ROUND_HD constexpr int kkt_tw_xch_doubles(int nd) { return 3 * nd * nd + 4 * nd; }
 
-enum ResultWord : int { RESULT_SWEEPS = 0, RESULT_IP_SOLVES = 1, RESULT_IP_ITERS = 2, RESULT_IP_FAILURES = 3, RESULT_NEWTON_SUM = 4 };
+enum ResultWord : int { RESULT_SWEEPS = 0, RESULT_IP_SOLVES = 1, RESULT_IP_ITERS = 2, RESULT_IP_FAILURES = 3, RESULT_NEWTON_SUM = 4,
+                        RESULT_IP_BEFORE = 5 };
 constexpr int RESULT_STATS = 4, RESULT_SUMS = 5, RESULT_HEADER = 8;
 ROUND_HD constexpr int result_record(int nu) { return nu + 2; }
 ROUND_HD constexpr size_t result_doubles(size_t B, int nu) { return RESULT_HEADER + B * (size_t)result_record(nu); }
```

New measurement: 75230, median of 6. Within noise of the previous version (+0.8%).
